# peterWon/D-LIOM

Measured on AMD Instinct MI355X. Metric: scans/sec (64-beam x 1024 pts -> 10 cm 3D submap), higher is better.
Workload: dtype f32 transforms + u16 voxels/u64 sums (rtcsm), f64 (ceres); 1 GPU; config2 W-dense: 64x1024 scan, all returns matched (adaptive voxel filters neutralised), RTCSM3D + CeresScanMatcher3D(hi+lo) + insertion(hi+lo); N_hi=65536, N_lo=65536, C=35937, linear_window=1, angular_window=5, rescored_candidates_last=2, box_kernel_variant=0, map_scans=20, grids_inserted_into=2, parallelism=replicas x1

## Files before the change

### d-liom_amd/csrc/rtcsm3d.hip

```cpp
#include <algorithm>
#include <cmath>
#include <cstdlib>
#include <cstring>
#include <type_traits>
#include <vector>

#include <dlfcn.h>
#include <rccl/rccl.h>

#include "device_common.h"
#include "host_math.h"
#include "probability_values.h"
#include "score_box.h"

namespace dliom {

constexpr int kBlock = 256;

template <int PPT, bool WIDE = false>
__global__ __launch_bounds__(kBlock) void rtcsm_score_kernel(
    GridView g, const float* __restrict__ px, const float* __restrict__ py,
    const float* __restrict__ pz, const float4* __restrict__ rot, int R, int r_first, int r_last,
    const float* __restrict__ trans, int T, int rots_per_block,
    unsigned long long* __restrict__ sums) {
  extern __shared__ unsigned block_sum[];
  float x[PPT], y[PPT], z[PPT];
#pragma unroll
  for (int k = 0; k < PPT; ++k) {
    const int i = (blockIdx.x * PPT + k) * kBlock + threadIdx.x;
    x[k] = px[i];
    y[k] = py[i];
    z[k] = pz[i];
  }
  const int r_begin = r_first + blockIdx.y * rots_per_block;
  const int r_end = min(r_begin + rots_per_block, r_last);
  const int lane = threadIdx.x & 63;
  const float inv = g.inv_resolution;
  typedef typename std::conditional<WIDE, unsigned long long, unsigned>::type idx_t;
  const idx_t sentinel = static_cast<idx_t>(1) << (3 * g.log2_leaves);
  const unsigned lb = static_cast<unsigned>(g.log2_leaves);
  for (int r = r_begin; r < r_end; ++r) {
    for (int j = threadIdx.x; j < T; j += kBlock) block_sum[j] = 0u;
    __syncthreads();
    const float4 qq = rot[r];
    const Quat4 q{qq.x, qq.y, qq.z, qq.w};
    float rx[PPT], ry[PPT], rz[PPT];
#pragma unroll
    for (int k = 0; k < PPT; ++k) rotate_point(q, x[k], y[k], z[k], rx[k], ry[k], rz[k]);
#pragma unroll 1
    for (int j = 0; j < T; ++j) {
      const float tx = trans[3 * j], ty = trans[3 * j + 1], tz = trans[3 * j + 2];
      idx_t tix[PPT];
      unsigned cel[PPT];
#pragma unroll
      for (int k = 0; k < PPT; ++k) {
        const float cx = rx[k] + tx, cy = ry[k] + ty, cz = rz[k] + tz;
        bool near = false;
        int ix = cell_fast(cx, inv, &near);
        int iy = cell_fast(cy, inv, &near);
        int iz = cell_fast(cz, inv, &near);
        if (__builtin_expect(near, 0)) {
          ix = cell_of(cx, g.resolution);
          iy = cell_of(cy, g.resolution);
          iz = cell_of(cz, g.resolution);
        }
        const unsigned sx = static_cast<unsigned>(ix + g.half);
        const unsigned sy = static_cast<unsigned>(iy + g.half);
        const unsigned sz = static_cast<unsigned>(iz + g.half);
        const bool inside = (sx | sy | sz) < g.grid_size;
        const idx_t t = (((static_cast<idx_t>(sz >> 3) << lb) | (sy >> 3)) << lb) | (sx >> 3);
        tix[k] = inside ? t : sentinel;
        cel[k] = ((sz & 7u) << 6) | ((sy & 7u) << 3) | (sx & 7u);
      }
#pragma unroll
      for (int k = 0; k < PPT; ++k) tix[k] = g.table[tix[k]];
#pragma unroll
      for (int k = 0; k < PPT; ++k) cel[k] = g.pool[(static_cast<size_t>(tix[k]) << 9) | cel[k]];
      unsigned a = 0;
#pragma unroll
      for (int k = 0; k < PPT; ++k) a += max(cel[k] & 0x7FFFu, 1u);
      const unsigned total = wave_sum_lane63(a);
      if (lane == 63) atomicAdd(&block_sum[j], total);
    }
    __syncthreads();
    for (int j = threadIdx.x; j < T; j += kBlock)
      atomicAdd(&sums[static_cast<size_t>(j) * R + r], static_cast<unsigned long long>(block_sum[j]));
  }
}

template <int TC, int P>
__global__ __launch_bounds__(kBlock) void rtcsm_score_rot_kernel(
    GridView g, const float* __restrict__ px, const float* __restrict__ py,
    const float* __restrict__ pz, int points_per_chunk, const float4* __restrict__ rot, int R,
    int r_first, int r_last, const float4* __restrict__ trans4, int T,
    unsigned long long* __restrict__ sums) {
  extern __shared__ float4 lds_trans[];
  __shared__ unsigned lds_acc[TC][kBlock];
  for (int j = threadIdx.x; j < T; j += kBlock) lds_trans[j] = trans4[j];
  __syncthreads();
  const int r = r_first + blockIdx.x * kBlock + threadIdx.x;
  const bool active = r < r_last;
  const float4 qq = rot[active ? r : r_first];
  const Quat4 q{qq.x, qq.y, qq.z, qq.w};
  const float inv = g.inv_resolution;
  const unsigned sentinel = 1u << (3 * g.log2_leaves);
  const unsigned lb = static_cast<unsigned>(g.log2_leaves);
  const int p_begin = blockIdx.y * points_per_chunk;
  const int p_end = p_begin + points_per_chunk;
  for (int jc = 0; jc < T; jc += TC) {
    const int tc = min(TC, T - jc);
    for (int jj = 0; jj < tc; ++jj) lds_acc[jj][threadIdx.x] = 0u;
#pragma unroll 1
    for (int i = p_begin; i < p_end; i += P) {
      float rx[P], ry[P], rz[P];
#pragma unroll
      for (int k = 0; k < P; ++k) rotate_point(q, px[i + k], py[i + k], pz[i + k], rx[k], ry[k], rz[k]);
#pragma unroll 1
      for (int jj = 0; jj < tc; ++jj) {
        const float4 t = lds_trans[jc + jj];
        unsigned tix[P], cel[P];
#pragma unroll
        for (int k = 0; k < P; ++k) {
          const float cx = rx[k] + t.x, cy = ry[k] + t.y, cz = rz[k] + t.z;
          bool near = false;
          int ix = cell_fast(cx, inv, &near);
          int iy = cell_fast(cy, inv, &near);
          int iz = cell_fast(cz, inv, &near);
          if (__builtin_expect(near, 0)) {
            ix = cell_of(cx, g.resolution);
            iy = cell_of(cy, g.resolution);
            iz = cell_of(cz, g.resolution);
          }
          const unsigned sx = static_cast<unsigned>(ix + g.half);
          const unsigned sy = static_cast<unsigned>(iy + g.half);
          const unsigned sz = static_cast<unsigned>(iz + g.half);
          const bool inside = (sx | sy | sz) < g.grid_size;
          const unsigned tt = (((sz >> 3) << lb | (sy >> 3)) << lb) | (sx >> 3);
          tix[k] = inside ? tt : sentinel;
          cel[k] = ((sz & 7u) << 6) | ((sy & 7u) << 3) | (sx & 7u);
        }
#pragma unroll
        for (int k = 0; k < P; ++k) tix[k] = g.table[tix[k]];
#pragma unroll
        for (int k = 0; k < P; ++k) cel[k] = g.pool[(tix[k] << 9) | cel[k]];
        unsigned a = 0;
#pragma unroll
        for (int k = 0; k < P; ++k) a += max(cel[k] & 0x7FFFu, 1u);
        atomicAdd(&lds_acc[jj][threadIdx.x], a);
      }
    }
    if (active) {
      for (int jj = 0; jj < tc; ++jj)
        atomicAdd(&sums[static_cast<size_t>(jc + jj) * R + r],
                  static_cast<unsigned long long>(lds_acc[jj][threadIdx.x]));
    }
  }
}

__device__ __forceinline__ int cvt_flr(float y) {
  int r;
  asm("v_cvt_flr_i32_f32 %0, %1" : "=v"(r) : "v"(y));
  return r;
}

constexpr int kDenseMaxBlock = 256;

struct DenseDomain {
  int lo;
  int size;
  int n_real;
  float pad[3];
};

template <bool CLAMP>
__global__ __launch_bounds__(kDenseMaxBlock) void rtcsm_score_dense_kernel(
    GridView g, DenseDomain dom, const float* __restrict__ px, const float* __restrict__ py,
    const float* __restrict__ pz, int points_per_chunk, int point_chunks,
    int rot_groups, const float4* __restrict__ rot, int R, int r_first, int r_last,
    const float4* __restrict__ trans4, int T, int t_chunk, unsigned long long* __restrict__ sums) {
  constexpr int P = 8;
  const int bs = blockDim.x;
  const int xcd = blockIdx.x & 7, slot = blockIdx.x >> 3;
  const int rot_group = slot % rot_groups;
  const int chunk_id = (slot / rot_groups) * 8 + xcd;
  if (chunk_id >= point_chunks) return;
  extern __shared__ float4 lds_dyn[];
  float4* lds_trans = lds_dyn;
  unsigned* lds_off = reinterpret_cast<unsigned*>(lds_dyn + T);
  const int S = g.dense_stride;
  const int TS = dom.size;
  unsigned* lds_acc = lds_off + 3 * TS;
  for (int j = threadIdx.x; j < T; j += bs) lds_trans[j] = trans4[j];
  {
    const unsigned B = static_cast<unsigned>(g.dense_bricks);
    for (int c = threadIdx.x; c < TS; c += bs) {
      const unsigned m = static_cast<unsigned>(min(max(c + dom.lo, 0), S - 1));
      const unsigned h = m >> 2, l = m & 3u;
      lds_off[c] = h * 128u + l * 2u;
      lds_off[TS + c] = h * B * 128u + l * 8u;
      lds_off[2 * TS + c] = h * B * B * 128u + l * 32u;
    }
  }
  __syncthreads();
  const int r = r_first + rot_group * bs + threadIdx.x;
  const bool active = r < r_last;
  const float4 qq = rot[active ? r : r_first];
  const Quat4 q{qq.x, qq.y, qq.z, qq.w};
  const float inv = g.inv_resolution;
  const float K = static_cast<float>(g.half + 1 - dom.lo) + 0.5f;
  const float band = 2.2f * static_cast<float>(TS) * 5.9604645e-8f;
  const float lim = static_cast<float>(TS - 1) + 0.5f;
  const int to_table = g.half + 1 - dom.lo;
  const int p_begin = chunk_id * points_per_chunk;
  const int p_end = p_begin + points_per_chunk;
  for (int jc = blockIdx.y * t_chunk; jc < T; jc += t_chunk * gridDim.y) {
    const int tc = min(t_chunk, T - jc);
    for (int jj = 0; jj < tc; ++jj) lds_acc[jj * bs + threadIdx.x] = 0u;
#pragma unroll 1
    for (int i = p_begin; i < p_end; i += P) {
      float rx[P], ry[P], rz[P];
#pragma unroll
      for (int k = 0; k < P; ++k) {
        const bool real = CLAMP || i + k < dom.n_real;
        rotate_point(q, real ? px[i + k] : dom.pad[0], real ? py[i + k] : dom.pad[1], real ? pz[i + k] : dom.pad[2],
                     rx[k], ry[k], rz[k]);
      }
#pragma unroll 1
      for (int jj = 0; jj < tc; ++jj) {
        const float4 t = lds_trans[jc + jj];
        unsigned ox[P], oy[P], oz[P];
        float lo[P], hi[P];
#pragma unroll
        for (int k = 0; k < P; ++k) {
          const float zx = __builtin_fmaf(rx[k] + t.x, inv, K), zy = __builtin_fmaf(ry[k] + t.y, inv, K),
                      zz = __builtin_fmaf(rz[k] + t.z, inv, K);
          const float fx = __builtin_amdgcn_fractf(zx), fy = __builtin_amdgcn_fractf(zy),
                      fz = __builtin_amdgcn_fractf(zz);
          lo[k] = fminf(fminf(fx, fy), fz);
          hi[k] = fmaxf(fmaxf(fx, fy), fz);
          if (CLAMP) {
            ox[k] = lds_off[cvt_flr(__builtin_amdgcn_fmed3f(zx, 0.f, lim))];
            oy[k] = lds_off[TS + cvt_flr(__builtin_amdgcn_fmed3f(zy, 0.f, lim))];
            oz[k] = lds_off[2 * TS + cvt_flr(__builtin_amdgcn_fmed3f(zz, 0.f, lim))];
          } else {
            ox[k] = lds_off[cvt_flr(zx)];
            oy[k] = lds_off[TS + cvt_flr(zy)];
            oz[k] = lds_off[2 * TS + cvt_flr(zz)];
          }
        }
        float m = lo[0], M = hi[0];
#pragma unroll
        for (int k = 1; k < P; ++k) {
          m = fminf(m, lo[k]);
          M = fmaxf(M, hi[k]);
        }
        if (__builtin_expect(m <= band || M >= 1.f - band, 0)) {
#pragma unroll
          for (int k = 0; k < P; ++k) {
            if (lo[k] <= band || hi[k] >= 1.f - band) {
              ox[k] = lds_off[min(max(cell_of(rx[k] + t.x, g.resolution) + to_table, 0), TS - 1)];
              oy[k] = lds_off[TS + min(max(cell_of(ry[k] + t.y, g.resolution) + to_table, 0), TS - 1)];
              oz[k] = lds_off[2 * TS + min(max(cell_of(rz[k] + t.z, g.resolution) + to_table, 0), TS - 1)];
            }
          }
        }
        unsigned v[P];
#pragma unroll
        for (int k = 0; k < P; ++k)
          v[k] = *reinterpret_cast<const unsigned short*>(reinterpret_cast<const char*>(g.dense) + (ox[k] + oy[k] + oz[k]));
        unsigned a = 0;
#pragma unroll
        for (int k = 0; k < P; ++k) a += v[k];
        atomicAdd(&lds_acc[jj * bs + threadIdx.x], a);
      }
    }
    if (active) {
      for (int jj = 0; jj < tc; ++jj)
        atomicAdd(&sums[static_cast<size_t>(jc + jj) * R + r],
                  static_cast<unsigned long long>(lds_acc[jj * bs + threadIdx.x]));
    }
  }
}

struct BoundParams {
  double a;
  double b;
  double delta;
  double wt, wr;
  int n;
  int n_pad;
  int R, T;
  int r_first, r_last;
};

__device__ double seq_sum_error_bound(int n, double U) {
  double err = 0.0;
  long long i = 0;
  for (int k = -4; k < 64 && i < n; ++k) {
    const double top = ldexp(1.0, k + 1);
    long long last;
    if (U < top) {
      last = n;
    } else {
      last = static_cast<long long>(floor(top / 0.93)) - 1;
      if (last > n) last = n;
    }
    if (last > i) {
      err += 0.5 * ldexp(1.0, k - 23) * static_cast<double>(last - i);
      i = last;
    }
  }
  return err;
}

__device__ __forceinline__ float next_up(float f) { return __uint_as_float(__float_as_uint(f) + 1u); }
__device__ __forceinline__ float next_down(float f) {
  const unsigned u = __float_as_uint(f);
  return u == 0u ? 0.f : __uint_as_float(u - 1u);
}

__global__ void rtcsm_bounds_kernel(const unsigned long long* __restrict__ sums, long long C,
                                    const float* __restrict__ t_norm, const float* __restrict__ r_angle,
                                    BoundParams p, float* __restrict__ lo, float* __restrict__ hi,
                                    unsigned* __restrict__ best_lo_bits) {
  const long long c = static_cast<long long>(blockIdx.x) * blockDim.x + threadIdx.x;
  const bool in_range = c < C;
  const int j = in_range ? static_cast<int>(c / p.R) : 0, r = in_range ? static_cast<int>(c % p.R) : 0;
  const bool mine = in_range && r >= p.r_first && r < p.r_last;
  float flo = 0.f, fhi = -1.f;
  if (mine) {
  const double s = static_cast<double>(sums[c] - static_cast<unsigned long long>(p.n_pad));
  const double mid = p.a * s + p.b * p.n;
  const double slack = p.delta * p.n + 1e-9 * mid;
  double sum_lo = mid - slack, sum_hi = mid + slack;
  const double U = sum_hi * (1.0 + 1.0 / 32.0);
  const double e = seq_sum_error_bound(p.n, U);
  if (sum_hi + e > U || p.n > (1 << 19)) {
    flo = 0.f;
    fhi = 3.0e38f;
  } else {
    sum_lo -= e;
    sum_hi += e;
    const double arg = static_cast<double>(t_norm[j]) * p.wt + static_cast<double>(r_angle[r]) * p.wr;
    const double pen = exp(-(arg * arg));
    const float nf = static_cast<float>(p.n);
    float qlo = next_down(next_down(static_cast<float>(sum_lo))) / nf;
    float qhi = next_up(next_up(static_cast<float>(sum_hi))) / nf;
    qlo = next_down(qlo);
    qhi = next_up(qhi);
    flo = next_down(next_down(static_cast<float>(static_cast<double>(qlo) * pen * (1.0 - 1e-9))));
    fhi = next_up(next_up(static_cast<float>(static_cast<double>(qhi) * pen * (1.0 + 1e-9))));
    if (!(flo > 0.f)) flo = 0.f;
  }
  }
  if (in_range) {
    lo[c] = flo;
    hi[c] = fhi;
  }
  unsigned best = __float_as_uint(flo);
#pragma unroll
  for (int off = 32; off > 0; off >>= 1) best = max(best, static_cast<unsigned>(__shfl_xor(static_cast<int>(best), off, 64)));
  if ((threadIdx.x & 63) == 0 && best != 0u) atomicMax(best_lo_bits, best);
}

__global__ void rtcsm_select_kernel(const float* __restrict__ hi, long long C,
                                    const unsigned* __restrict__ best_lo_bits,
                                    unsigned* __restrict__ count, unsigned* __restrict__ list) {
  const long long c = static_cast<long long>(blockIdx.x) * blockDim.x + threadIdx.x;
  if (c >= C) return;
  const float best_lo = __uint_as_float(*best_lo_bits);
  if (hi[c] >= best_lo) {
    const unsigned k = atomicAdd(count, 1u);
    list[k] = static_cast<unsigned>(c);
  }
}

__global__ void probe_cells_kernel(Quat4 q, float tx, float ty, float tz, const float* __restrict__ px,
                                   const float* __restrict__ py, const float* __restrict__ pz, int n,
                                   float resolution, int* __restrict__ out) {
  const int i = blockIdx.x * blockDim.x + threadIdx.x;
  if (i >= n) return;
  float rx, ry, rz;
  rotate_point(q, px[i], py[i], pz[i], rx, ry, rz);
  out[3 * i] = cell_of(rx + tx, resolution);
  out[3 * i + 1] = cell_of(ry + ty, resolution);
  out[3 * i + 2] = cell_of(rz + tz, resolution);
}

struct Candidates {
  dliom_rtcsm_window w;
  PoseF init;
  std::vector<QF> rot;
  std::vector<QF> rot_raw;
  std::vector<float> r_angle;
  std::vector<F3> trans;
  std::vector<float> t_norm;
};

static void compute_window(const dliom_rtcsm_options& o, float resolution, float cloud_max_norm_value,
                           dliom_rtcsm_window* w) {
  w->linear_window_size = static_cast<int>(std::lround(o.linear_search_window / resolution));
  float max_scan_range = 3.f * resolution;
  max_scan_range = std::max(cloud_max_norm_value, max_scan_range);
  const float kSafetyMargin = 1.f - 1e-3f;
  const float res2 = resolution * (resolution * 1.f);
  const float range2 = max_scan_range * (max_scan_range * 1.f);
  w->angular_step_size = kSafetyMargin * std::acos(1.f - res2 / (2.f * range2));
  w->angular_window_size =
      static_cast<int>(std::lround(o.angular_search_window / w->angular_step_size));
  w->max_scan_range = max_scan_range;
  const int64_t tl = 2 * static_cast<int64_t>(w->linear_window_size) + 1;
  const int64_t ta = 2 * static_cast<int64_t>(w->angular_window_size) + 1;
  w->num_translations = tl * tl * tl;
  w->num_rotations = ta * ta * ta;
  w->num_candidates = w->num_translations * w->num_rotations;
}

static void generate_candidates(const dliom_rtcsm_options& o, float resolution, float max_norm,
                                const double init7[7], Candidates* c) {
  compute_window(o, resolution, max_norm, &c->w);
  c->init.t = F3{static_cast<float>(init7[0]), static_cast<float>(init7[1]), static_cast<float>(init7[2])};
  c->init.q = QF{static_cast<float>(init7[3]), static_cast<float>(init7[4]),
                 static_cast<float>(init7[5]), static_cast<float>(init7[6])};
  const int L = c->w.linear_window_size, A = c->w.angular_window_size;
  const float step = c->w.angular_step_size;
  struct RotCache {
    int A = -1;
    float step = 0.f;
    std::vector<QF> rot_raw;
    std::vector<float> r_angle;
  };
  static thread_local RotCache cache;
  if (cache.A != A || cache.step != step) {
    cache.A = A;
    cache.step = step;
    cache.rot_raw.clear();
    cache.r_angle.clear();
    cache.rot_raw.reserve(c->w.num_rotations);
    cache.r_angle.reserve(c->w.num_rotations);
    for (int rz = -A; rz <= A; ++rz)
      for (int ry = -A; ry <= A; ++ry)
        for (int rx = -A; rx <= A; ++rx) {
          const QF q = angle_axis_to_quaternion(F3{rx * step, ry * step, rz * step});
          cache.rot_raw.push_back(q);
          cache.r_angle.push_back(rotation_angle(q));
        }
  }
  c->rot_raw = cache.rot_raw;
  c->r_angle = cache.r_angle;
  c->rot.resize(cache.rot_raw.size());
  for (size_t i = 0; i < cache.rot_raw.size(); ++i) c->rot[i] = qnormalized(qmul(c->init.q, cache.rot_raw[i]));
  c->trans.clear();
  c->t_norm.clear();
  for (int z = -L; z <= L; ++z)
    for (int y = -L; y <= L; ++y)
      for (int x = -L; x <= L; ++x) {
        const F3 t{x * resolution, y * resolution, z * resolution};
        c->t_norm.push_back(norm3(t));
        c->trans.push_back(add3(qrot(c->init.q, t), c->init.t));
      }
}

struct DeviceCandidates {
  float4* rot;
  float* trans;
  float4* trans4;
  float* t_norm;
  float* r_angle;
  const float4* rot_src;
};

static bool prep_add(PrepArgs* prep, void* dst, const void* src, size_t bytes, unsigned value) {
  if (prep == nullptr || prep->n >= kMaxPrepJobs || (bytes & 3u) != 0 || (reinterpret_cast<uintptr_t>(dst) & 15u) != 0 ||
      (reinterpret_cast<uintptr_t>(src) & 15u) != 0 || bytes / 16 > 0xFFFFFFFFull)
    return false;
  PrepJob& j = prep->job[prep->n++];
  j.dst = static_cast<uint4*>(dst);
  j.src = static_cast<const uint4*>(src);
  j.vec = static_cast<unsigned>(bytes / 16);
  j.tail_words = static_cast<unsigned>((bytes % 16) / 4);
  j.value = value;
  return true;
}
__global__ __launch_bounds__(256) void rtcsm_prep_kernel(PrepArgs a) { prep_block(a, blockIdx.x, gridDim.x, threadIdx.x, blockDim.x); }
static int prep_flush(dliom_ctx* ctx, PrepArgs* prep) {
  if (prep == nullptr || prep->n == 0) return DLIOM_OK;
  unsigned most = 1;
  for (int j = 0; j < prep->n; ++j) most = std::max(most, prep->job[j].vec);
  hipLaunchKernelGGL(rtcsm_prep_kernel, dim3(std::min(512u, (most + 255u) / 256u)), dim3(256), 0, ctx->stream, *prep);
  DLIOM_HIP_TRY(hipGetLastError());
  prep->n = 0;
  return DLIOM_OK;
}

static int upload_candidates(dliom_ctx* ctx, const Candidates& c, DeviceCandidates* d, PrepArgs* prep = nullptr) {
  const size_t R = c.rot.size(), T = c.trans.size();
  const size_t Tpad = T;
  const size_t bytes_rot = align256(R * 16);
  const size_t bytes_trans = align256(Tpad * 12);
  const size_t bytes_tn = align256(T * 4);
  const size_t bytes_ra = align256(R * 4);
  const size_t bytes_t4 = align256(T * 16);
  const size_t total = bytes_rot + bytes_trans + bytes_tn + bytes_ra + bytes_t4;
  DLIOM_TRY(ctx->cand.reserve(total));
  std::vector<char> host(total, 0);
  float* hr = reinterpret_cast<float*>(host.data());
  for (size_t i = 0; i < R; ++i) {
    hr[4 * i] = c.rot[i].w;
    hr[4 * i + 1] = c.rot[i].x;
    hr[4 * i + 2] = c.rot[i].y;
    hr[4 * i + 3] = c.rot[i].z;
  }
  float* ht = reinterpret_cast<float*>(host.data() + bytes_rot);
  for (size_t i = 0; i < Tpad; ++i) {
    const F3& t = c.trans[std::min(i, T - 1)];
    ht[3 * i] = t.x;
    ht[3 * i + 1] = t.y;
    ht[3 * i + 2] = t.z;
  }
  std::memcpy(host.data() + bytes_rot + bytes_trans, c.t_norm.data(), T * 4);
  std::memcpy(host.data() + bytes_rot + bytes_trans + bytes_tn, c.r_angle.data(), R * 4);
  float* h4 = reinterpret_cast<float*>(host.data() + bytes_rot + bytes_trans + bytes_tn + bytes_ra);
  for (size_t i = 0; i < T; ++i) {
    h4[4 * i] = c.trans[i].x;
    h4[4 * i + 1] = c.trans[i].y;
    h4[4 * i + 2] = c.trans[i].z;
    h4[4 * i + 3] = 0.f;
  }
  char* base = static_cast<char*>(ctx->cand.p);
  d->rot_src = reinterpret_cast<const float4*>(base);
  if (total <= kPinRtcsmCandidates.bytes) {
    void* staged = pinned_at(ctx, kPinRtcsmCandidates);
    std::memcpy(staged, host.data(), total);
    if (prep_add(prep, base, staged, total, 0u))
      d->rot_src = static_cast<const float4*>(staged);
    else
      DLIOM_HIP_TRY(hipMemcpyAsync(base, staged, total, hipMemcpyHostToDevice, ctx->stream));
  } else {
    DLIOM_HIP_TRY(hipMemcpyAsync(base, host.data(), total, hipMemcpyHostToDevice, ctx->stream));
    DLIOM_HIP_TRY(hipStreamSynchronize(ctx->stream));
  }
  d->rot = reinterpret_cast<float4*>(base);
  d->trans = reinterpret_cast<float*>(base + bytes_rot);
  d->t_norm = reinterpret_cast<float*>(base + bytes_rot + bytes_trans);
  d->r_angle = reinterpret_cast<float*>(base + bytes_rot + bytes_trans + bytes_tn);
  d->trans4 = reinterpret_cast<float4*>(base + bytes_rot + bytes_trans + bytes_tn + bytes_ra);
  return DLIOM_OK;
}

static int env_int(const char* name, int fallback) { return tuning_int(name, fallback); }

static int launch_score_box(dliom_ctx* ctx, const dliom_cloud& cloud, const GridView& g, const Candidates& c,
                            const DeviceCandidates& d, int r_first, int r_last, unsigned long long* d_sums,
                            unsigned* d_error, PrepArgs* prep) {
  using namespace box;
  const int R = static_cast<int>(c.w.num_rotations), T = static_cast<int>(c.w.num_translations);
  const int n = static_cast<int>(cloud.n);
  static const int forced_variant = env_int("DLIOM_BOX_VARIANT", -1);
  const auto padded = [T](int tc) { return ((T + tc - 1) / tc) * tc; };
  const int variant = forced_variant >= 0 && forced_variant <= 2
                          ? forced_variant
                          : (T <= kTC ? 0 : (0.87 * padded(kTCWide) < 0.9 * padded(kTC) ? 2 : 1));
  const int TC = variant == 2 ? kTCWide : kTC;
  static const int forced_cells = env_int("DLIOM_BOX_CELLS", 0);
  const int cells = forced_cells > 0 ? forced_cells : (variant == 0 ? 14336 : 21000);
  static const int forced_chunk = env_int("DLIOM_BOX_CHUNK", 0);
  const int chunk_pts = forced_chunk > 0 ? forced_chunk : (variant == 0 ? kCostChunk : kCostChunkBig);
  const double res = static_cast<double>(g.resolution);
  const int passes = (T + TC - 1) / TC;
  double tmax = 0.0;
  for (const F3& t : c.trans) tmax = std::max(tmax, static_cast<double>(std::max(std::fabs(t.x), std::max(std::fabs(t.y), std::fabs(t.z)))));
  const double rmax = static_cast<double>(cloud.max_norm) / res + 1.0;
  const double qmax = rmax + tmax / res + 1.0;
  if (!std::isfinite(qmax) || qmax > 16500.0) return (ctx->last_box_refusal = DLIOM_BOX_REFUSED_RANGE, DLIOM_ERR_CAPACITY);
  std::vector<Pass> pass(static_cast<size_t>(passes));
  std::vector<float> tau(static_cast<size_t>(passes) * TC * 4, 0.f);
  double taumax = 0.0;
  for (int tp = 0; tp < passes; ++tp) {
    const int j0 = tp * TC, tc = std::min(TC, T - j0);
    for (int a = 0; a < 3; ++a) {
      double lo = 1e300, hi = -1e300;
      for (int j = j0; j < j0 + tc; ++j) {
        const double v = a == 0 ? c.trans[j].x : (a == 1 ? c.trans[j].y : c.trans[j].z);
        lo = std::min(lo, v);
        hi = std::max(hi, v);
      }
      taumax = std::max(taumax, (hi - lo) * 0.5 / res + 1.0);
    }
  }
  if (rmax + taumax + 130.0 > 1000.0) return (ctx->last_box_refusal = DLIOM_BOX_REFUSED_RANGE, DLIOM_ERR_CAPACITY);
  const double e16 = 1.0 + (2.0 * qmax + rmax + taumax) / 256.0;
  const int B = static_cast<int>(std::ceil(e16 + 0.25));
  const int s_units = B;
  const double u = 1.0 / 65536.0;
  for (int tp = 0; tp < passes; ++tp) {
    Pass& ps = pass[static_cast<size_t>(tp)];
    ps.j0 = tp * TC;
    ps.tc = std::min(TC, T - ps.j0);
    ps.pad[0] = ps.pad[1] = 0;
    for (int a = 0; a < 3; ++a) {
      auto comp = [&](int j) { return static_cast<double>(a == 0 ? c.trans[j].x : (a == 1 ? c.trans[j].y : c.trans[j].z)); };
      double lo = 1e300, hi = -1e300;
      for (int j = ps.j0; j < ps.j0 + ps.tc; ++j) {
        lo = std::min(lo, comp(j));
        hi = std::max(hi, comp(j));
      }
      const double tcen = 0.5 * (lo + hi);
      const double G = tcen / res + 128.5 + s_units * u;
      const double gi = std::floor(G);
      const double f = std::nearbyint((G - gi) * 16384.0) / 16384.0;
      ps.gi[a] = static_cast<int>(gi);
      ps.f[a] = static_cast<float>(f);
      ps.uc[a] = static_cast<float>(tcen / res + 0.5);
      double reach = 0.0;
      for (int jj = 0; jj < TC; ++jj) {
        const int j = ps.j0 + std::min(jj, ps.tc - 1);
        const double tv = comp(j) / res + 128.5 + s_units * u - (gi + f);
        const float tf = static_cast<float>(tv);
        tau[(static_cast<size_t>(tp) * TC + jj) * 4 + a] = tf;
        reach = std::max(reach, std::fabs(static_cast<double>(tf)));
      }
      ps.reach[a] = static_cast<float>(reach + 0.02 + qmax * std::ldexp(1.0, -22));
    }
  }
  std::vector<unsigned> bitmap(static_cast<size_t>(passes) * kBitmapWords, 0u);
  const unsigned thr_units = static_cast<unsigned>(s_units + B);
  for (int tp = 0; tp < passes; ++tp) {
    const Pass& ps = pass[static_cast<size_t>(tp)];
    for (int a = 0; a < 3; ++a) {
      unsigned* words = bitmap.data() + static_cast<size_t>(tp) * kBitmapWords + static_cast<size_t>(a) * (kBuckets / 32);
      for (int jj = 0; jj < ps.tc; ++jj) {
        const double tv = static_cast<double>(tau[(static_cast<size_t>(tp) * TC + jj) * 4 + a]);
        const double af = tv - std::floor(tv);
        const double L = -af - 1.5 * u, H = -af + (thr_units + 1.5) * u;
        const long long b0 = static_cast<long long>(std::floor(L * kBuckets)), b1 = static_cast<long long>(std::floor(H * kBuckets));
        for (long long b = b0; b <= b1; ++b) {
          const unsigned m = static_cast<unsigned>(((b % kBuckets) + kBuckets) % kBuckets);
          words[m >> 5] |= 1u << (m & 31u);
        }
      }
    }
  }
  {
    const double step = c.w.angular_step_size;
    const double a_lanes = (2.0 * c.w.angular_window_size + 1.0) * step;
    const double spread = a_lanes * 0.6 * cloud.max_norm / res;
    const double dim = spread + 2.0 * taumax + 8.0;
    if (dim > kMaxDim || dim * dim * (dim * 0.25) > cells) return (ctx->last_box_refusal = DLIOM_BOX_REFUSED_WINDOW, DLIOM_ERR_CAPACITY);
  }
  const int rot_groups_all = (r_last - r_first + 63) / 64;
  static const int forced_nw = env_int("DLIOM_BOX_NW", 0);
  const int nw = forced_nw >= 1 && forced_nw <= kWaves
                     ? std::min(forced_nw, rot_groups_all)
                     : std::min(rot_groups_all, kWaves);
  const int rot_blocks = (rot_groups_all + nw - 1) / nw;
  if (TC * sizeof(float4) + kBitmapWords * 4 + 16 + static_cast<size_t>(nw) * kListWords * 4 + static_cast<size_t>(cells) * 2 >
      160 * 1024)
    return (ctx->last_box_refusal = DLIOM_BOX_REFUSED_LDS, DLIOM_ERR_CAPACITY);
  struct GroupCache {
    int A = -1, r_first = -1, r_last = -1, nw = 0;
    float step = 0.f;
    std::vector<Group> groups;
  };
  static thread_local GroupCache gcache;
  const bool gcache_hit = gcache.A == c.w.angular_window_size && gcache.step == c.w.angular_step_size &&
                          gcache.r_first == r_first && gcache.r_last == r_last && gcache.nw == nw;
  std::vector<Group>& groups = gcache.groups;
  if (!gcache_hit) {
    gcache.A = -1;
    groups.assign(static_cast<size_t>(rot_blocks), Group());
  }
  for (size_t gi = 0; !gcache_hit && gi < groups.size(); ++gi) {
    Group& gr = groups[gi];
    const int r0 = r_first + static_cast<int>(gi) * nw * 64;
    const int cnt = std::max(0, std::min(nw * 64, r_last - r0));
    gr.c_lane = cnt / 2;
    gr.theta2 = 0.f;
    for (int a = 0; a < 3; ++a) gr.dc[a] = gr.hd[a] = 0.f;
    if (cnt <= 0) {
      gr.c_lane = 0;
      continue;
    }
    auto qd = [&](int r, double q[4]) {
      const QF& f = c.rot_raw[static_cast<size_t>(r)];
      const double nn = std::sqrt(double(f.w) * f.w + double(f.x) * f.x + double(f.y) * f.y + double(f.z) * f.z);
      q[0] = f.w / nn; q[1] = f.x / nn; q[2] = f.y / nn; q[3] = f.z / nn;
    };
    double qc[4];
    qd(r0 + gr.c_lane, qc);
    double lo3[3] = {1e300, 1e300, 1e300}, hi3[3] = {-1e300, -1e300, -1e300}, th = 0.0;
    for (int l = 0; l < cnt; ++l) {
      double q[4];
      qd(r0 + l, q);
      const double a0 = qc[0], a1 = -qc[1], a2 = -qc[2], a3 = -qc[3];
      double dq[4] = {a0 * q[0] - a1 * q[1] - a2 * q[2] - a3 * q[3], a0 * q[1] + a1 * q[0] + a2 * q[3] - a3 * q[2],
                      a0 * q[2] - a1 * q[3] + a2 * q[0] + a3 * q[1], a0 * q[3] + a1 * q[2] - a2 * q[1] + a3 * q[0]};
      if (dq[0] < 0) for (double& v : dq) v = -v;
      const double vn = std::sqrt(dq[1] * dq[1] + dq[2] * dq[2] + dq[3] * dq[3]);
      const double ang = 2.0 * std::atan2(vn, dq[0]);
      const double k = vn > 1e-300 ? ang / vn : 2.0;
      const double dv[3] = {k * dq[1], k * dq[2], k * dq[3]};
      th = std::max(th, ang);
      for (int a = 0; a < 3; ++a) {
        lo3[a] = std::min(lo3[a], dv[a]);
        hi3[a] = std::max(hi3[a], dv[a]);
      }
    }
    if (th > 0.3) return (ctx->last_box_refusal = DLIOM_BOX_REFUSED_WINDOW, DLIOM_ERR_CAPACITY);
    for (int a = 0; a < 3; ++a) {
      gr.dc[a] = static_cast<float>(0.5 * (lo3[a] + hi3[a]));
      gr.hd[a] = static_cast<float>(0.5 * (hi3[a] - lo3[a]) * 1.0001 + 1e-7);
    }
    gr.theta2 = static_cast<float>(0.51 * th * th * 1.01 + 1e-9);
  }
  gcache.A = c.w.angular_window_size;
  gcache.step = c.w.angular_step_size;
  gcache.r_first = r_first;
  gcache.r_last = r_last;
  gcache.nw = nw;
  struct SpanGuard {
    dliom_ctx* c;
    int span;
    ~SpanGuard() { c->end_span(span); }
  } span_guard{ctx, ctx->begin_span(DLIOM_KERNEL_RTCSM_SCORE)};
  const size_t tau_bytes = align256(tau.size() * 4);
  const size_t pass_only_bytes = align256(pass.size() * sizeof(Pass));
  const size_t group_bytes = align256(groups.size() * sizeof(Group));
  const size_t bitmap_bytes = align256(bitmap.size() * 4);
  const size_t pass_bytes = pass_only_bytes + group_bytes + bitmap_bytes;
  DLIOM_TRY(ctx->box_tables.reserve(tau_bytes + pass_bytes));
  char* base = static_cast<char*>(ctx->box_tables.p);
  const Group* group_src = reinterpret_cast<const Group*>(base + tau_bytes + pass_only_bytes);
  if (tau_bytes + pass_bytes <= kPinBoxTables.bytes) {
    char* h = pinned_at<char>(ctx, kPinBoxTables);
    std::memcpy(h, tau.data(), tau.size() * 4);
    std::memcpy(h + tau_bytes, pass.data(), pass.size() * sizeof(Pass));
    std::memcpy(h + tau_bytes + pass_only_bytes, groups.data(), groups.size() * sizeof(Group));
    std::memcpy(h + tau_bytes + pass_only_bytes + group_bytes, bitmap.data(), bitmap.size() * 4);
    if (prep_add(prep, base, h, tau_bytes + pass_bytes, 0u))
      group_src = reinterpret_cast<const Group*>(h + tau_bytes + pass_only_bytes);
    else
      DLIOM_HIP_TRY(hipMemcpyAsync(base, h, tau_bytes + pass_bytes, hipMemcpyHostToDevice, ctx->stream));
  } else {
    DLIOM_HIP_TRY(hipMemcpyAsync(base, tau.data(), tau.size() * 4, hipMemcpyHostToDevice, ctx->stream));
    DLIOM_HIP_TRY(hipMemcpyAsync(base + tau_bytes, pass.data(), pass.size() * sizeof(Pass), hipMemcpyHostToDevice, ctx->stream));
    DLIOM_HIP_TRY(hipMemcpyAsync(base + tau_bytes + pass_only_bytes, groups.data(), groups.size() * sizeof(Group),
                                 hipMemcpyHostToDevice, ctx->stream));
    DLIOM_HIP_TRY(hipMemcpyAsync(base + tau_bytes + pass_only_bytes + group_bytes, bitmap.data(), bitmap.size() * 4,
                                 hipMemcpyHostToDevice, ctx->stream));
    DLIOM_HIP_TRY(hipStreamSynchronize(ctx->stream));
  }
  Params p;
  p.tau = reinterpret_cast<const float4*>(base);
  p.pass = reinterpret_cast<const Pass*>(base + tau_bytes);
  p.group = reinterpret_cast<const Group*>(base + tau_bytes + pass_only_bytes);
  p.bitmap = reinterpret_cast<const unsigned*>(base + tau_bytes + pass_only_bytes + group_bytes);
  p.trans = d.trans;
  p.rot = d.rot;
  p.sums = d_sums;
  p.error = d_error;
  p.R = R;
  p.r_first = r_first;
  p.r_last = r_last;
  p.T = T;
  p.passes = passes;
  p.n = n;
  p.chunk = std::min(kMaxChunk, std::max(4, chunk_pts & ~3));
  p.order = p.chunk == kCostChunk ? cloud.d_chunk_order : (p.chunk == kCostChunkBig ? cloud.d_chunk_order_big : nullptr);
  p.point_chunks = (n + p.chunk - 1) / p.chunk;
  const int rot_groups = (r_last - r_first + 63) / 64;
  p.rot_groups = rot_groups;
  p.rot_blocks = rot_blocks;
  p.nw = nw;
  p.thr = thr_units;
  p.cells = cells;
  static const int split_points = env_int("DLIOM_BOX_SPLIT", 1);
  p.split_points = split_points;
#ifdef DLIOM_EXPERIMENTS
  static const int box_debug = env_int("DLIOM_BOX_DEBUG", 0);
  p.debug = box_debug;
  if (box_debug & 512) p.order = nullptr;
#else
  p.debug = 0;
#endif
  const size_t lds = TC * sizeof(float4) + kBitmapWords * 4 + 16 + static_cast<size_t>(nw) * kListWords * 4 +
                     static_cast<size_t>(cells) * 2;
  if (lds > 160 * 1024) return (ctx->last_box_refusal = DLIOM_BOX_REFUSED_LDS, DLIOM_ERR_CAPACITY);
  typedef void (*BoxKernel)(GridView, Params, const float*, const float*, const float*);
  const BoxKernel kernel = variant == 0 ? rtcsm_score_box_kernel : (variant == 1 ? rtcsm_score_box_kernel_w3 : rtcsm_score_box_kernel_wide);
  const unsigned attr_bit = variant == 0 ? kFuncAttrScoreBox : (variant == 1 ? kFuncAttrScoreBoxW3 : kFuncAttrScoreBoxWide);
  if ((ctx->func_attr_set & attr_bit) == 0u) {
    DLIOM_HIP_TRY(hipFuncSetAttribute(reinterpret_cast<const void*>(kernel), hipFuncAttributeMaxDynamicSharedMemorySize, 160 * 1024));
    ctx->func_attr_set |= attr_bit;
  }
  ctx->last_box_variant = variant;
  static thread_local size_t resident_lds = 0;
  static thread_local int resident = 0, resident_nw = 0, resident_variant = -1;
  if (resident_lds != lds || resident_nw != nw || resident_variant != variant) {
    resident_nw = nw;
    resident_variant = variant;
    DLIOM_HIP_TRY(hipOccupancyMaxActiveBlocksPerMultiprocessor(&resident, reinterpret_cast<const void*>(kernel), 64 * nw, lds));
    resident_lds = lds;
  }
  const int want_blocks = std::max(1, resident) * ctx->num_cus;
  int slot_quads = std::max(1, want_blocks / std::max(1, rot_blocks * passes));
  slot_quads = std::min(slot_quads, p.point_chunks);
  p.slots = slot_quads;
  p.units = passes * rot_blocks;
  DLIOM_TRY(ctx->box_counters.reserve(static_cast<size_t>(passes) * rot_blocks * 4 + 256));
  if (!prep_add(prep, ctx->box_counters.p, nullptr, static_cast<size_t>(passes) * rot_blocks * 4, 0u))
    DLIOM_HIP_TRY(hipMemsetAsync(ctx->box_counters.p, 0, static_cast<size_t>(passes) * rot_blocks * 4, ctx->stream));
  p.counters = ctx->box_counters.as<unsigned>();
  p.ext_stride = static_cast<int>(cloud.n_padded);
  DLIOM_TRY(ctx->box_extents.reserve(static_cast<size_t>(rot_blocks) * 6 * static_cast<size_t>(cloud.n_padded) * 4));
  p.ext = ctx->box_extents.as<float>();
  {
    PrepArgs none;
    none.n = 0;
    const PrepArgs& jobs = prep != nullptr ? *prep : none;
    const unsigned prep_rows = jobs.n > 0 ? 1u : 0u;
    hipLaunchKernelGGL(rtcsm_box_extent_kernel, dim3(static_cast<unsigned>((n + 255) / 256), static_cast<unsigned>(rot_blocks) + prep_rows),
                       dim3(256), 0, ctx->stream, p, g.inv_resolution, cloud.d_xs, cloud.d_ys, cloud.d_zs, ctx->box_extents.as<float>(),
                       group_src, d.rot_src, jobs);
    if (prep != nullptr) prep->n = 0;
  }
  const unsigned blocks = static_cast<unsigned>(slot_quads) * passes * rot_blocks;
  hipLaunchKernelGGL(kernel, dim3(blocks), dim3(64 * nw), lds, ctx->stream, g, p, cloud.d_xs, cloud.d_ys, cloud.d_zs);
  DLIOM_HIP_TRY(hipGetLastError());
#ifdef DLIOM_TEST_HOOKS
  if (ctx->tuning[DLIOM_TUNE_RESERVED_TEST_HOOK] == 1) {
    ctx->tuning[DLIOM_TUNE_RESERVED_TEST_HOOK] = 0;
    DLIOM_HIP_TRY(hipMemsetAsync(static_cast<char*>(ctx->box_error.p) + 4, 1, 1, ctx->stream));
  }
#endif
  return DLIOM_OK;
}

constexpr int kScoreTargetBlocks = 8192;

static int launch_score_dense(dliom_ctx* ctx, const dliom_cloud& cloud, const GridView& g, const Candidates& c,
                              const DeviceCandidates& d, int r_first, int r_last, unsigned long long* d_sums,
                              int64_t* processed) {
  const int R = static_cast<int>(c.w.num_rotations), T = static_cast<int>(c.w.num_translations);
  const int n = static_cast<int>(cloud.n);
  const int Rs = r_last - r_first;
  const size_t trans_lds = static_cast<size_t>(T) * 16;
  if (trans_lds > 100 * 1024) return DLIOM_ERR_INVALID_ARGUMENT;
  int bs = kDenseMaxBlock;
  for (int cand = kDenseMaxBlock; cand >= 64; cand -= 64)
    if ((Rs + cand - 1) / cand * cand < (Rs + bs - 1) / bs * bs) bs = cand;
  if (static_cast<int64_t>((Rs + bs - 1) / bs) * ((n + 63) / 64) < 256) bs = 64;
  const int rot_groups = (Rs + bs - 1) / bs;
  int chunk = 4096;
  while (chunk > 8 && static_cast<int64_t>(rot_groups) * ((n + chunk - 1) / chunk) < kScoreTargetBlocks) chunk >>= 1;
  const int point_chunks = (n + chunk - 1) / chunk;
  *processed = static_cast<int64_t>(point_chunks) * chunk;
  DenseDomain dom;
  dom.lo = 0;
  dom.size = g.dense_stride;
  dom.n_real = n;
  dom.pad[0] = dom.pad[1] = dom.pad[2] = kPadCoordinate;
  bool clamp = true;
  {
    float tmax = 0.f, t_init = norm3(c.init.t);
    for (const F3& t : c.trans) tmax = std::max(tmax, std::max(std::fabs(t.x), std::max(std::fabs(t.y), std::fabs(t.z))));
    const float res = g.resolution;
    const double reach = (static_cast<double>(cloud.max_norm) + tmax) / res + 3.0;
    const double theta_max = 1.7321 * (c.w.angular_window_size + 1) * c.w.angular_step_size * 1.01 + 1e-4;
    const double rho = (g.half + 64) * static_cast<double>(res) + t_init;
    const double m_cells = 8.0 + std::ceil((theta_max * rho + (c.w.linear_window_size + 1) * res * 1.7321) / res);
    const double hi_cell = std::max(reach, g.half + 2.0 * m_cells);
    const int lo_i = std::min(0, g.half + 1 - static_cast<int>(std::ceil(hi_cell)));
    const int hi_i = std::max(g.dense_stride, g.half + 1 + static_cast<int>(std::ceil(hi_cell)) + 1);
    if (m_cells <= 64.0 && hi_i - lo_i <= 1024 && std::isfinite(reach)) {
      clamp = false;
      dom.lo = lo_i;
      dom.size = hi_i - lo_i;
      const F3 w{static_cast<float>((g.half + m_cells) * res) - c.init.t.x, -c.init.t.y, -c.init.t.z};
      const QF qi{c.init.q.w, -c.init.q.x, -c.init.q.y, -c.init.q.z};
      const F3 p = qrot(qi, w);
      dom.pad[0] = p.x;
      dom.pad[1] = p.y;
      dom.pad[2] = p.z;
    }
  }
  const size_t fixed_lds = trans_lds + static_cast<size_t>(dom.size) * 12;
  const size_t acc_budget = fixed_lds < 34 * 1024 ? 36 * 1024 - fixed_lds : 2 * 1024;
  int t_chunk = std::max(4, std::min(std::min(T, 27), static_cast<int>(acc_budget / (static_cast<size_t>(bs) * 4))));
  const int chunks_per_xcd = (point_chunks + 7) / 8;
  int t_slices = 1;
  const int base_blocks = 8 * chunks_per_xcd * rot_groups;
  if (base_blocks < 512 && T > 1) {
    const int want = std::min(T, (1024 + base_blocks - 1) / base_blocks);
    t_chunk = std::min(t_chunk, (T + want - 1) / want);
    t_slices = (T + t_chunk - 1) / t_chunk;
  }
  const size_t lds = fixed_lds + static_cast<size_t>(t_chunk) * bs * 4;
  const auto kernel = clamp ? &rtcsm_score_dense_kernel<true> : &rtcsm_score_dense_kernel<false>;
  const int span = ctx->begin_span(DLIOM_KERNEL_RTCSM_SCORE);
  hipLaunchKernelGGL(kernel, dim3(base_blocks, t_slices), dim3(bs), lds, ctx->stream, g, dom, cloud.d_xs, cloud.d_ys,
                     cloud.d_zs, chunk, point_chunks, rot_groups, d.rot, R, r_first, r_last, d.trans4, T, t_chunk, d_sums);
  ctx->end_span(span);
  return DLIOM_OK;
}

static int launch_score_rot(dliom_ctx* ctx, const dliom_cloud& cloud, const GridView& g, const Candidates& c,
                            const DeviceCandidates& d, int r_first, int r_last, unsigned long long* d_sums,
                            int64_t* processed) {
  const int R = static_cast<int>(c.w.num_rotations), T = static_cast<int>(c.w.num_translations);
  const int n = static_cast<int>(cloud.n);
  const size_t lds = static_cast<size_t>(T) * 16;
  if (lds > 100 * 1024) return DLIOM_ERR_INVALID_ARGUMENT;
  const int rot_groups = (r_last - r_first + kBlock - 1) / kBlock;
  int chunk = 4096;
  while (chunk > 64 && static_cast<int64_t>(rot_groups) * ((n + chunk - 1) / chunk) < kScoreTargetBlocks) chunk >>= 1;
  const int point_chunks = (n + chunk - 1) / chunk;
  *processed = static_cast<int64_t>(point_chunks) * chunk;
  const auto kernel = T == 1 ? &rtcsm_score_rot_kernel<1, 4> : &rtcsm_score_rot_kernel<27, 8>;
  const int span = ctx->begin_span(DLIOM_KERNEL_RTCSM_SCORE);
  hipLaunchKernelGGL(kernel, dim3(rot_groups, point_chunks), dim3(kBlock), lds, ctx->stream, g, cloud.d_xs, cloud.d_ys,
                     cloud.d_zs, chunk, d.rot, R, r_first, r_last, d.trans4, T, d_sums);
  ctx->end_span(span);
  return DLIOM_OK;
}

static int launch_score_point(dliom_ctx* ctx, const dliom_cloud& cloud, const GridView& g, const Candidates& c,
                              const DeviceCandidates& d, int r_first, int r_last, unsigned long long* d_sums,
                              int64_t* processed) {
  const int R = static_cast<int>(c.w.num_rotations), T = static_cast<int>(c.w.num_translations);
  const int n = static_cast<int>(cloud.n);
  const int Rs = r_last - r_first;
  int ppt = n >= 32 * 1024 ? 8 : (n >= 8 * 1024 ? 4 : (n >= 2048 ? 2 : 1));
  while (ppt > 1 && (cloud.n_padded % (static_cast<int64_t>(kBlock) * ppt)) != 0) ppt >>= 1;
  const int point_tiles = (n + kBlock * ppt - 1) / (kBlock * ppt);
  int rot_tiles = std::max(1, std::min(Rs, (kScoreTargetBlocks + point_tiles - 1) / point_tiles));
  const int rots_per_block = (Rs + rot_tiles - 1) / rot_tiles;
  rot_tiles = (Rs + rots_per_block - 1) / rots_per_block;
  const size_t lds = static_cast<size_t>(T) * sizeof(unsigned);
  if (lds > 150 * 1024) return DLIOM_ERR_INVALID_ARGUMENT;
  const bool wide = g.log2_leaves > 10;
  const int lane_pts = wide ? (ppt >= 4 ? 4 : 1) : ppt;
  const int tile = kBlock * lane_pts;
  const int tiles = (n + tile - 1) / tile;
  *processed = static_cast<int64_t>(tiles) * tile;
  auto kernel = &rtcsm_score_kernel<1>;
  if (wide) kernel = lane_pts == 4 ? &rtcsm_score_kernel<4, true> : &rtcsm_score_kernel<1, true>;
  else if (lane_pts == 8) kernel = &rtcsm_score_kernel<8>;
  else if (lane_pts == 4) kernel = &rtcsm_score_kernel<4>;
  else if (lane_pts == 2) kernel = &rtcsm_score_kernel<2>;
  const int span = ctx->begin_span(DLIOM_KERNEL_RTCSM_SCORE);
  hipLaunchKernelGGL(kernel, dim3(tiles, rot_tiles), dim3(kBlock), lds, ctx->stream, g, cloud.d_xs, cloud.d_ys, cloud.d_zs,
                     d.rot, R, r_first, r_last, d.trans, T, rots_per_block, d_sums);
  ctx->end_span(span);
  return DLIOM_OK;
}

static int run_score_volume(dliom_ctx* ctx, const dliom_cloud& cloud, const dliom_grid* grid,
                            const Candidates& c, int r_first, int r_last, DeviceCandidates* d,
                            unsigned long long** d_sums, int64_t* pad_processed, const FillJob* also_fill = nullptr) {
  PrepArgs prep;
  prep.n = 0;
  DLIOM_TRY(upload_candidates(ctx, c, d, &prep));
  const int64_t C = c.w.num_candidates;
  DLIOM_TRY(ctx->sums.reserve(static_cast<size_t>(C) * 8));
  *d_sums = ctx->sums.as<unsigned long long>();
  {
    FillJob fills[2] = {{*d_sums, static_cast<size_t>(C) * 8, 0u}, {nullptr, 0, 0u}};
    int nf = 1;
    if (also_fill != nullptr) fills[nf++] = *also_fill;
    for (int k = 0; k < nf; ++k)
      if (!prep_add(&prep, fills[k].p, nullptr, fills[k].bytes, fills[k].value)) DLIOM_TRY(fill_multi(ctx, &fills[k], 1));
  }
  const int T = static_cast<int>(c.w.num_translations);
  const int n = static_cast<int>(cloud.n);
  int mapping = ctx->tuning[DLIOM_TUNE_SCORE_KERNEL];
  ctx->last_box_refusal = mapping == 3 ? DLIOM_BOX_RAN : DLIOM_BOX_NOT_REQUESTED;
  if (ctx->force_dense_score && mapping > 2) {
    mapping = 2;
    ctx->last_box_refusal = DLIOM_BOX_REFUSED_FLAGGED;
  }
  ctx->last_score_used_box = false;
  if (mapping >= 2) {
    const float res = grid->resolution;
    const int centre[3] = {static_cast<int>(std::lround(c.init.t.x / res)), static_cast<int>(std::lround(c.init.t.y / res)),
                           static_cast<int>(std::lround(c.init.t.z / res))};
    const double reach_cells = static_cast<double>(cloud.max_norm) / res + (c.w.linear_window_size + 1) * 1.7321 + 4.0;
    const int radius = reach_cells < 1.0e6 ? static_cast<int>(std::ceil(reach_cells)) : (1 << 20);
    if (const_cast<dliom_grid*>(grid)->ensure_dense_for(centre, radius) != DLIOM_OK) {
      if (mapping == 3) ctx->last_box_refusal = DLIOM_BOX_REFUSED_NO_MIRROR;
      mapping = 1;
    }
  }
  const bool windowed = grid->dense_windowed;
  if (windowed && mapping == 2) mapping = 1;
  const GridView g = grid->view();
  DLIOM_TRY(ensure_morton(ctx, &cloud));
  if (g.log2_leaves > 10 && mapping >= 1) {
    if (mapping == 3) ctx->last_box_refusal = DLIOM_BOX_REFUSED_NO_MIRROR;
    mapping = 0;
  }
  if (mapping == 3) {
    const double pairs = static_cast<double>(C) * static_cast<double>(n);
    int s3 = DLIOM_ERR_CAPACITY;
    ctx->last_box_refusal = DLIOM_BOX_REFUSED_SMALL;
    if (T >= 8 && pairs >= std::ldexp(1.0, 24)) {
      ctx->last_box_refusal = DLIOM_BOX_RAN;
#ifdef DLIOM_EXPERIMENTS
      constexpr size_t kBoxErrorBytes = 256 + 4096 * 32;
#else
      constexpr size_t kBoxErrorBytes = 256;
#endif
      DLIOM_TRY(ctx->box_error.reserve(kBoxErrorBytes));
      if (!ctx->box_error_zeroed) {
        DLIOM_HIP_TRY(hipMemsetAsync(ctx->box_error.p, 0, kBoxErrorBytes, ctx->stream));
        ctx->box_error_zeroed = true;
      }
      s3 = launch_score_box(ctx, cloud, g, c, *d, r_first, r_last, *d_sums, ctx->box_error.as<unsigned>(), &prep);
    }
    if (s3 == DLIOM_OK) {
      *pad_processed = 0;
      ctx->last_score_used_box = true;
      ctx->last_score_mapping = 3;
      return DLIOM_OK;
    }
    if (s3 != DLIOM_ERR_CAPACITY) return s3;
    mapping = windowed ? 1 : 2;
  }
  DLIOM_TRY(prep_flush(ctx, &prep));
  ctx->last_score_mapping = mapping;
  int64_t processed = 0;
  if (mapping == 2)
    DLIOM_TRY(launch_score_dense(ctx, cloud, g, c, *d, r_first, r_last, *d_sums, &processed));
  else if (mapping == 1)
    DLIOM_TRY(launch_score_rot(ctx, cloud, g, c, *d, r_first, r_last, *d_sums, &processed));
  else
    DLIOM_TRY(launch_score_point(ctx, cloud, g, c, *d, r_first, r_last, *d_sums, &processed));
  DLIOM_HIP_TRY(hipGetLastError());
  *pad_processed = processed - n;
  return DLIOM_OK;
}

struct LutModel {
  double a, b, delta;
};
static const LutModel& lut_model() {
  static const LutModel m = [] {
    LutModel r;
    r.a = static_cast<double>(kValueToProbabilityScale);
    r.b = static_cast<double>(kValueToProbabilityOffset);
    double d = std::fabs(static_cast<double>(kUnknownProbability) - (r.a * 1.0 + r.b));
    for (int v = 1; v < 32768; ++v) {
      const float f = v * kValueToProbabilityScale + kValueToProbabilityOffset;
      d = std::max(d, std::fabs(static_cast<double>(f) - (r.a * v + r.b)));
    }
    r.delta = d * 1.0000001 + 1e-12;
    return r;
  }();
  return m;
}

struct RtcsmState {
  dliom_rtcsm_options o;
  Candidates c;
  DeviceCandidates d;
  dliom_cloud cloud;
  const dliom_grid* grid = nullptr;
  int r_first = 0, r_last = 0;
  unsigned long long* d_sums = nullptr;
  float* d_hi = nullptr;
  unsigned* d_list = nullptr;
  unsigned* d_ctrs = nullptr;
  float best_score = -1.f;
  int64_t best_c = -1;
  bool active = false;
  double init7[7] = {0, 0, 0, 1, 0, 0, 0};
  int shard = 0, num_shards = 1;
  bool used_box = false;
};

static int box_overflowed(dliom_ctx* ctx, unsigned err1, bool* overflow) {
  *overflow = err1 != 0u;
  if (*overflow)
    DLIOM_HIP_TRY(hipMemsetAsync(static_cast<char*>(ctx->box_error.p) + 4, 0, 4, ctx->stream));
  return DLIOM_OK;
}

static RtcsmState* state_of(dliom_ctx* ctx) {
  if (ctx->rtcsm_state == nullptr) {
    ctx->rtcsm_state = new RtcsmState;
    ctx->rtcsm_state_free = [](void* p) { delete static_cast<RtcsmState*>(p); };
  }
  return static_cast<RtcsmState*>(ctx->rtcsm_state);
}

static int match_begin(dliom_ctx* ctx, const dliom_rtcsm_options* o, const double init7[7],
                       const dliom_cloud& cloud, const dliom_grid* grid, int shard, int num_shards,
                       unsigned* local_best_lo_bits) {
  if (cloud.n <= 0) return DLIOM_ERR_EMPTY_CLOUD;
  if (cloud.n > (1 << 27) || num_shards < 1 || shard < 0 || shard >= num_shards)
    return DLIOM_ERR_INVALID_ARGUMENT;
  RtcsmState* st = state_of(ctx);
  st->active = false;
  st->o = *o;
  st->cloud = cloud;
  st->grid = grid;
  std::memcpy(st->init7, init7, sizeof st->init7);
  st->shard = shard;
  st->num_shards = num_shards;
  st->used_box = false;
  Candidates& c = st->c;
  generate_candidates(*o, grid->resolution, cloud.max_norm, init7, &c);
  const int64_t C = c.w.num_candidates;
  const int R = static_cast<int>(c.w.num_rotations), T = static_cast<int>(c.w.num_translations);
  if (C <= 0 || C > (int64_t{1} << 31)) return DLIOM_ERR_INVALID_ARGUMENT;
  st->r_first = static_cast<int>(static_cast<int64_t>(R) * shard / num_shards);
  st->r_last = static_cast<int>(static_cast<int64_t>(R) * (shard + 1) / num_shards);

  const size_t bytes_f = align256(static_cast<size_t>(C) * 4);
  DLIOM_TRY(ctx->bounds.reserve(3 * bytes_f + 256));
  char* bb = static_cast<char*>(ctx->bounds.p);
  float* d_lo = reinterpret_cast<float*>(bb);
  st->d_hi = reinterpret_cast<float*>(bb + bytes_f);
  st->d_list = reinterpret_cast<unsigned*>(bb + 2 * bytes_f);
  st->d_ctrs = reinterpret_cast<unsigned*>(bb + 3 * bytes_f);
  const FillJob zero_ctrs{st->d_ctrs, 8, 0u};
  if (st->r_last <= st->r_first) DLIOM_TRY(fill_multi(ctx, &zero_ctrs, 1));
  if (st->r_last > st->r_first) {
    int64_t pad_processed = 0;
    DLIOM_TRY(run_score_volume(ctx, cloud, grid, c, st->r_first, st->r_last, &st->d, &st->d_sums,
                               &pad_processed, &zero_ctrs));
    st->used_box = ctx->last_score_used_box;
    const LutModel& lm = lut_model();
    BoundParams bp;
    bp.a = lm.a;
    bp.b = lm.b;
    bp.delta = lm.delta;
    bp.wt = o->translation_delta_cost_weight;
    bp.wr = o->rotation_delta_cost_weight;
    bp.n = static_cast<int>(cloud.n);
    bp.n_pad = static_cast<int>(pad_processed);
    bp.R = R;
    bp.T = T;
    bp.r_first = st->r_first;
    bp.r_last = st->r_last;
    const unsigned cblocks = static_cast<unsigned>((C + 255) / 256);
    const int span = ctx->begin_span(DLIOM_KERNEL_RTCSM_SELECT);
    hipLaunchKernelGGL(rtcsm_bounds_kernel, dim3(cblocks), dim3(256), 0, ctx->stream, st->d_sums,
                       static_cast<long long>(C), st->d.t_norm, st->d.r_angle, bp, d_lo, st->d_hi,
                       st->d_ctrs);
    ctx->end_span(span);
    DLIOM_HIP_TRY(hipGetLastError());
  }
  if (local_best_lo_bits != nullptr) {
    unsigned* h_err = pinned_at<unsigned>(ctx, kPinBoxErrorWord);
    *h_err = 0u;
    DLIOM_HIP_TRY(hipMemcpyAsync(local_best_lo_bits, st->d_ctrs, 4, hipMemcpyDeviceToHost, ctx->stream));
    if (st->used_box)
      DLIOM_HIP_TRY(hipMemcpyAsync(h_err, static_cast<char*>(ctx->box_error.p) + 4, 4, hipMemcpyDeviceToHost, ctx->stream));
    DLIOM_HIP_TRY(hipStreamSynchronize(ctx->stream));
    bool overflow = false;
    DLIOM_TRY(box_overflowed(ctx, *h_err, &overflow));
    if (overflow && !ctx->force_dense_score) {
      ctx->force_dense_score = true;
      const dliom_rtcsm_options o_copy = st->o;
      const int s = match_begin(ctx, &o_copy, init7, cloud, grid, shard, num_shards, local_best_lo_bits);
      ctx->force_dense_score = false;
      return s;
    }
  }
  st->active = true;
  return DLIOM_OK;
}

static int match_finish(dliom_ctx* ctx, const unsigned* global_best_lo_bits, uint64_t* local_best_packed) {
  RtcsmState* st = state_of(ctx);
  if (!st->active) return DLIOM_ERR_INVALID_ARGUMENT;
  const dliom_rtcsm_options* o = &st->o;
  const Candidates& c = st->c;
  const int64_t C = c.w.num_candidates;
  const int R = static_cast<int>(c.w.num_rotations);
  const dliom_cloud& cloud = st->cloud;
  st->best_score = -1.f;
  st->best_c = -1;
  unsigned K = 0;
  if (st->r_last > st->r_first) {
    if (global_best_lo_bits != nullptr) {
      DLIOM_HIP_TRY(hipMemcpyAsync(st->d_ctrs, global_best_lo_bits, 4, hipMemcpyHostToDevice, ctx->stream));
    }
    const unsigned cblocks = static_cast<unsigned>((C + 255) / 256);
    int span = ctx->begin_span(DLIOM_KERNEL_RTCSM_SELECT);
    hipLaunchKernelGGL(rtcsm_select_kernel, dim3(cblocks), dim3(256), 0, ctx->stream, st->d_hi,
                       static_cast<long long>(C), st->d_ctrs, st->d_ctrs + 1, st->d_list);
    ctx->end_span(span);
    DLIOM_HIP_TRY(hipGetLastError());
  }
  constexpr unsigned kSpecK = 8;
  std::vector<unsigned> list;
  std::vector<float> ksums;
  if (st->r_last > st->r_first) {
    static_assert((2 + 2 * kSpecK + 1) * 4 <= kPinMatchReadback.bytes, "the read-back fits its region");
    unsigned* h_ctrs = pinned_at<unsigned>(ctx, kPinMatchReadback);
    unsigned* h_list = h_ctrs + 2;
    float* h_sums = reinterpret_cast<float*>(h_ctrs + 2 + kSpecK);
    auto rescore = [&](unsigned count, const unsigned* d_count, size_t list_offset) -> int {
      DLIOM_TRY(ctx->rescore.reserve(align256(static_cast<size_t>(count) * 4)));
      const int span = ctx->begin_span(DLIOM_KERNEL_RTCSM_RESCORE);
      const int s = launch_sequential_sums(ctx, sequential_sum_method(cloud.n), st->grid->view(), cloud, st->d.rot, R, st->d.trans,
                                           st->d_list + list_offset, d_count, count, &ctx->misc, ctx->rescore.as<float>());
      ctx->end_span(span);
      return s;
    };
    DLIOM_TRY(rescore(kSpecK, st->d_ctrs + 1, 0));
    unsigned* h_err = h_ctrs + 2 + 2 * kSpecK;
    *h_err = 0u;
    const bool want_err = st->used_box && global_best_lo_bits == nullptr;
    const GatherJob back[4] = {{st->d_ctrs, 2}, {st->d_list, kSpecK}, {ctx->rescore.p, kSpecK},
                               {static_cast<char*>(ctx->box_error.p) + 4, 1}};
    DLIOM_TRY(gather_and_wait(ctx, back, want_err ? 4 : 3, h_ctrs));
    {
      bool overflow = false;
      DLIOM_TRY(box_overflowed(ctx, *h_err, &overflow));
      if (overflow && !ctx->force_dense_score) {
        ctx->force_dense_score = true;
        const dliom_rtcsm_options o_copy = st->o;
        const dliom_cloud cloud_copy = st->cloud;
        double init_copy[7];
        std::memcpy(init_copy, st->init7, sizeof init_copy);
        int s = match_begin(ctx, &o_copy, init_copy, cloud_copy, st->grid, st->shard, st->num_shards, nullptr);
        if (s == DLIOM_OK) s = match_finish(ctx, nullptr, local_best_packed);
        ctx->force_dense_score = false;
        return s;
      }
    }
    K = h_ctrs[1];
    const unsigned first = std::min(K, kSpecK);
    list.assign(h_list, h_list + first);
    ksums.assign(h_sums, h_sums + first);
    if (K > kSpecK) {
      const unsigned rest = K - kSpecK;
      DLIOM_TRY(rescore(rest, nullptr, kSpecK));
      list.resize(K);
      ksums.resize(K);
      DLIOM_HIP_TRY(hipMemcpyAsync(list.data() + kSpecK, st->d_list + kSpecK, static_cast<size_t>(rest) * 4,
                                   hipMemcpyDeviceToHost, ctx->stream));
      DLIOM_HIP_TRY(hipMemcpyAsync(ksums.data() + kSpecK, ctx->rescore.p, static_cast<size_t>(rest) * 4,
                                   hipMemcpyDeviceToHost, ctx->stream));
      DLIOM_HIP_TRY(hipStreamSynchronize(ctx->stream));
    }
  }
  if (K > 0) {
    const int n = static_cast<int>(cloud.n);
    for (unsigned k = 0; k < K; ++k) {
      const int64_t cc = list[k];
      const int j = static_cast<int>(cc / R), r = static_cast<int>(cc % R);
      float score = ksums[k];
      score /= static_cast<float>(n);
      const double arg = c.t_norm[j] * o->translation_delta_cost_weight +
                         c.r_angle[r] * o->rotation_delta_cost_weight;
      score *= std::exp(-(arg * (arg * 1.0)));
      if (score > st->best_score || (score == st->best_score && cc < st->best_c)) {
        st->best_score = score;
        st->best_c = cc;
      }
    }
  }
  ctx->last_rtcsm.window = c.w;
  ctx->last_rtcsm.num_points = cloud.n;
  ctx->last_rtcsm.num_rescored = K;
  ctx->last_rtcsm.score_kernel = ctx->last_score_mapping;
  ctx->last_rtcsm.box_kernel_status = ctx->last_box_refusal;
  ctx->last_rtcsm.box_kernel_variant = ctx->last_box_refusal == DLIOM_BOX_RAN ? ctx->last_box_variant : -1;
  ctx->last_rtcsm.best_index = st->best_c;
  if (local_best_packed != nullptr) {
    uint64_t packed = 0;
    if (st->best_c >= 0 && st->best_score > 0.f) {
      uint32_t bits;
      std::memcpy(&bits, &st->best_score, 4);
      packed = (static_cast<uint64_t>(bits) << 32) | (0xFFFFFFFFull - static_cast<uint64_t>(st->best_c));
    }
    *local_best_packed = packed;
  }
  return DLIOM_OK;
}

static int match_decode(dliom_ctx* ctx, uint64_t best_packed, double out7[7], float* out_score) {
  RtcsmState* st = state_of(ctx);
  if (!st->active) return DLIOM_ERR_INVALID_ARGUMENT;
  if (best_packed == 0) return DLIOM_ERR_SCORE_NOT_POSITIVE;
  const Candidates& c = st->c;
  const int R = static_cast<int>(c.w.num_rotations);
  const uint32_t bits = static_cast<uint32_t>(best_packed >> 32);
  const int64_t best_c = static_cast<int64_t>(0xFFFFFFFFull - (best_packed & 0xFFFFFFFFull));
  if (best_c < 0 || best_c >= c.w.num_candidates) return DLIOM_ERR_INVALID_ARGUMENT;
  float score;
  std::memcpy(&score, &bits, 4);
  const int j = static_cast<int>(best_c / R), r = static_cast<int>(best_c % R);
  out7[0] = c.trans[j].x;
  out7[1] = c.trans[j].y;
  out7[2] = c.trans[j].z;
  out7[3] = c.rot[r].w;
  out7[4] = c.rot[r].x;
  out7[5] = c.rot[r].y;
  out7[6] = c.rot[r].z;
  *out_score = score;
  ctx->last_rtcsm.best_index = best_c;
  return DLIOM_OK;
}

static int match_impl(dliom_ctx* ctx, const dliom_rtcsm_options* o, const double init7[7],
                      const dliom_cloud& cloud, const dliom_grid* grid, double out7[7],
                      float* out_score) {
  DLIOM_TRY(match_begin(ctx, o, init7, cloud, grid, 0, 1, nullptr));
  uint64_t packed = 0;
  DLIOM_TRY(match_finish(ctx, nullptr, &packed));
  return match_decode(ctx, packed, out7, out_score);
}

}

using namespace dliom;

extern "C" {

int dliom_rtcsm3d_window(const dliom_rtcsm_options* o, float resolution, const float* points_xyz,
                         int64_t n, dliom_rtcsm_window* w) {
  if (o == nullptr || w == nullptr || n < 0 || (n > 0 && points_xyz == nullptr))
    return DLIOM_ERR_INVALID_ARGUMENT;
  compute_window(*o, resolution, cloud_max_norm(points_xyz, n), w);
  return DLIOM_OK;
}

int dliom_rtcsm3d_match_cloud(dliom_ctx* ctx, const dliom_rtcsm_options* o, const double init7[7],
                              const dliom_cloud* cloud, const dliom_grid* grid, double out7[7],
                              float* score) {
  if (ctx == nullptr || o == nullptr || init7 == nullptr || cloud == nullptr || grid == nullptr ||
      out7 == nullptr || score == nullptr)
    return DLIOM_ERR_INVALID_ARGUMENT;
  DLIOM_HIP_TRY(hipSetDevice(ctx->device));
  return match_impl(ctx, o, init7, *cloud, grid, out7, score);
}

int dliom_rtcsm3d_match(dliom_ctx* ctx, const dliom_rtcsm_options* o, const double init7[7],
                        const float* points_xyz, int64_t n, const dliom_grid* grid, double out7[7],
                        float* score) {
  if (ctx == nullptr || o == nullptr || init7 == nullptr || grid == nullptr || out7 == nullptr ||
      score == nullptr || n < 0 || (n > 0 && points_xyz == nullptr))
    return DLIOM_ERR_INVALID_ARGUMENT;
  if (n == 0) return DLIOM_ERR_EMPTY_CLOUD;
  DLIOM_HIP_TRY(hipSetDevice(ctx->device));
  DLIOM_TRY(ctx->points.reserve(staged_cloud_bytes(n)));
  dliom_cloud cloud;
  DLIOM_TRY(stage_cloud(ctx, points_xyz, n, &cloud));
  return match_impl(ctx, o, init7, cloud, grid, out7, score);
}

int dliom_rtcsm3d_shard_begin(dliom_ctx* ctx, const dliom_rtcsm_options* o, const double init7[7],
                              const dliom_cloud* cloud, const dliom_grid* grid, int shard, int num_shards,
                              uint32_t* local_best_lower_bound_bits) {
  if (ctx == nullptr || o == nullptr || init7 == nullptr || cloud == nullptr || grid == nullptr ||
      local_best_lower_bound_bits == nullptr)
    return DLIOM_ERR_INVALID_ARGUMENT;
  DLIOM_HIP_TRY(hipSetDevice(ctx->device));
  return match_begin(ctx, o, init7, *cloud, grid, shard, num_shards, local_best_lower_bound_bits);
}

int dliom_rtcsm3d_shard_finish(dliom_ctx* ctx, uint32_t global_best_lower_bound_bits,
                               uint64_t* local_best_packed) {
  if (ctx == nullptr || local_best_packed == nullptr) return DLIOM_ERR_INVALID_ARGUMENT;
  DLIOM_HIP_TRY(hipSetDevice(ctx->device));
  return match_finish(ctx, &global_best_lower_bound_bits, local_best_packed);
}

int dliom_rtcsm3d_shard_decode(dliom_ctx* ctx, uint64_t global_best_packed, double pose_estimate[7],
                               float* score) {
  if (ctx == nullptr || pose_estimate == nullptr || score == nullptr) return DLIOM_ERR_INVALID_ARGUMENT;
  return match_decode(ctx, global_best_packed, pose_estimate, score);
}

static constexpr uint64_t kShardFailed = 0x7FFFFFFFFFFFFFFFull;
int dliom_rtcsm3d_match_sharded(dliom_ctx* ctx, const dliom_rtcsm_options* o, const double init7[7], const dliom_cloud* cloud,
                                const dliom_grid* grid, int shard, int num_shards, dliom_allreduce_max_u64 exchange,
                                void* user, double out7[7], float* score) {
  if (num_shards > 1 && exchange == nullptr) return DLIOM_ERR_INVALID_ARGUMENT;
  int local = ctx == nullptr || o == nullptr || init7 == nullptr || cloud == nullptr || grid == nullptr || out7 == nullptr ||
                      score == nullptr
                  ? DLIOM_ERR_INVALID_ARGUMENT
                  : DLIOM_OK;
  if (local == DLIOM_OK && hipSetDevice(ctx->device) != hipSuccess) local = DLIOM_ERR_HIP;
  uint64_t packed = 0;
  if (local == DLIOM_OK) local = match_begin(ctx, o, init7, *cloud, grid, shard, num_shards, nullptr);
  if (local == DLIOM_OK) local = match_finish(ctx, nullptr, &packed);
  if (local != DLIOM_OK) packed = kShardFailed;
  if (num_shards > 1 && exchange(&packed, user) != 0) return local != DLIOM_OK ? local : DLIOM_ERR_HIP;
  if (local != DLIOM_OK) return local;
  if (packed == kShardFailed) return DLIOM_ERR_PEER_FAILED;
  return match_decode(ctx, packed, out7, score);
}

}

namespace {
struct RcclApi {
  ncclResult_t (*CommCount)(const ncclComm_t, int*) = nullptr;
  ncclResult_t (*CommUserRank)(const ncclComm_t, int*) = nullptr;
  ncclResult_t (*AllReduce)(const void*, void*, size_t, ncclDataType_t, ncclRedOp_t, ncclComm_t, hipStream_t) = nullptr;
  bool ok = false;
};
const RcclApi& rccl_api() {
  static const RcclApi api = [] {
    RcclApi a;
    void* h = dlopen("librccl.so.1", RTLD_NOW | RTLD_GLOBAL);
    if (h == nullptr) h = dlopen("librccl.so", RTLD_NOW | RTLD_GLOBAL);
    if (h == nullptr) return a;
    a.CommCount = reinterpret_cast<decltype(a.CommCount)>(dlsym(h, "ncclCommCount"));
    a.CommUserRank = reinterpret_cast<decltype(a.CommUserRank)>(dlsym(h, "ncclCommUserRank"));
    a.AllReduce = reinterpret_cast<decltype(a.AllReduce)>(dlsym(h, "ncclAllReduce"));
    a.ok = a.CommCount != nullptr && a.CommUserRank != nullptr && a.AllReduce != nullptr;
    return a;
  }();
  return api;
}
struct RcclExchange {
  dliom_ctx* ctx;
  ncclComm_t comm;
};
int rccl_exchange(uint64_t* value, void* user) {
  RcclExchange* x = static_cast<RcclExchange*>(user);
  dliom_ctx* ctx = x->ctx;
  if (ctx->misc.reserve(256) != DLIOM_OK) return 1;
  uint64_t* d = ctx->misc.as<uint64_t>();
  uint64_t* h = pinned_at<uint64_t>(ctx, kPinRcclWord);
  *h = *value;
  const int span = ctx->begin_span(DLIOM_KERNEL_ALLREDUCE);
  bool ok = hipMemcpyAsync(d, h, 8, hipMemcpyHostToDevice, ctx->stream) == hipSuccess &&
            rccl_api().AllReduce(d, d, 1, ncclUint64, ncclMax, x->comm, ctx->stream) == ncclSuccess &&
            hipMemcpyAsync(h, d, 8, hipMemcpyDeviceToHost, ctx->stream) == hipSuccess;
  ctx->end_span(span);
  if (!ok) return 1;
  if (hipStreamSynchronize(ctx->stream) != hipSuccess) return 1;
  *value = *h;
  return 0;
}
}

extern "C" {

int dliom_rtcsm3d_match_sharded_rccl(dliom_ctx* ctx, const dliom_rtcsm_options* o, const double init7[7],
                                     const dliom_cloud* cloud, const dliom_grid* grid, void* nccl_comm, double out7[7],
                                     float* score) {
  if (ctx == nullptr || nccl_comm == nullptr) return DLIOM_ERR_INVALID_ARGUMENT;
  const RcclApi& api = rccl_api();
  if (!api.ok) {
    set_last_error("dlopen(librccl.so.1): RCCL not available", hipErrorSharedObjectInitFailed, __FILE__, __LINE__);
    return DLIOM_ERR_HIP;
  }
  int rank = 0, size = 1;
  ncclComm_t comm = static_cast<ncclComm_t>(nccl_comm);
  if (api.CommCount(comm, &size) != ncclSuccess || api.CommUserRank(comm, &rank) != ncclSuccess) return DLIOM_ERR_INVALID_ARGUMENT;
  RcclExchange x{ctx, comm};
  if (size == 1) {
    if (ctx == nullptr || o == nullptr || init7 == nullptr || cloud == nullptr || grid == nullptr || out7 == nullptr ||
        score == nullptr)
      return DLIOM_ERR_INVALID_ARGUMENT;
    int local = hipSetDevice(ctx->device) == hipSuccess ? DLIOM_OK : DLIOM_ERR_HIP;
    uint64_t packed = 0;
    if (local == DLIOM_OK) local = match_begin(ctx, o, init7, *cloud, grid, 0, 1, nullptr);
    if (local == DLIOM_OK) local = match_finish(ctx, nullptr, &packed);
    if (local != DLIOM_OK) packed = kShardFailed;
    if (rccl_exchange(&packed, &x) != 0) return local != DLIOM_OK ? local : DLIOM_ERR_HIP;
    if (local != DLIOM_OK) return local;
    return match_decode(ctx, packed, out7, score);
  }
  return dliom_rtcsm3d_match_sharded(ctx, o, init7, cloud, grid, rank, size, rccl_exchange, &x, out7, score);
}

int dliom_rtcsm3d_box_error(dliom_ctx* ctx, uint32_t* flags) {
  if (ctx == nullptr || flags == nullptr) return DLIOM_ERR_INVALID_ARGUMENT;
  *flags = 0;
  if (ctx->box_error.p == nullptr) return DLIOM_OK;
  DLIOM_HIP_TRY(hipSetDevice(ctx->device));
  DLIOM_HIP_TRY(hipMemcpyAsync(flags, ctx->box_error.p, 4, hipMemcpyDeviceToHost, ctx->stream));
  DLIOM_HIP_TRY(hipStreamSynchronize(ctx->stream));
  return DLIOM_OK;
}

#ifdef DLIOM_EXPERIMENTS
extern "C" int dliom_exp_box_stats(dliom_ctx* ctx, uint32_t out[8]) {
  if (ctx == nullptr || out == nullptr || ctx->box_error.p == nullptr) return DLIOM_ERR_INVALID_ARGUMENT;
  DLIOM_HIP_TRY(hipMemcpyAsync(out, static_cast<char*>(ctx->box_error.p) + 32, 32, hipMemcpyDeviceToHost, ctx->stream));
  DLIOM_HIP_TRY(hipMemsetAsync(static_cast<char*>(ctx->box_error.p) + 32, 0, 32, ctx->stream));
  DLIOM_HIP_TRY(hipStreamSynchronize(ctx->stream));
  return DLIOM_OK;
}
#endif

#ifdef DLIOM_EXPERIMENTS
extern "C" int dliom_exp_box_stamps(dliom_ctx* ctx, uint64_t* out, int workgroups) {
  if (ctx == nullptr || out == nullptr || ctx->box_error.p == nullptr || workgroups > 4096) return DLIOM_ERR_INVALID_ARGUMENT;
  DLIOM_HIP_TRY(hipMemcpyAsync(out, static_cast<char*>(ctx->box_error.p) + 256, static_cast<size_t>(workgroups) * 32,
                               hipMemcpyDeviceToHost, ctx->stream));
  DLIOM_HIP_TRY(hipStreamSynchronize(ctx->stream));
  return DLIOM_OK;
}
#endif

int dliom_rtcsm3d_last_stats(const dliom_ctx* ctx, dliom_rtcsm_stats* stats) {
  if (ctx == nullptr || stats == nullptr) return DLIOM_ERR_INVALID_ARGUMENT;
  *stats = ctx->last_rtcsm;
  return DLIOM_OK;
}

int dliom_rtcsm3d_score_volume(dliom_ctx* ctx, const dliom_rtcsm_options* o, const double init7[7],
                               const float* points_xyz, int64_t n, const dliom_grid* grid,
                               uint64_t* sums, int64_t capacity, int64_t* num_candidates) {
  if (ctx == nullptr || o == nullptr || init7 == nullptr || grid == nullptr ||
      num_candidates == nullptr || n <= 0 || points_xyz == nullptr)
    return DLIOM_ERR_INVALID_ARGUMENT;
  DLIOM_HIP_TRY(hipSetDevice(ctx->device));
  DLIOM_TRY(ctx->points.reserve(staged_cloud_bytes(n)));
  dliom_cloud cloud;
  DLIOM_TRY(stage_cloud(ctx, points_xyz, n, &cloud));
  Candidates c;
  generate_candidates(*o, grid->resolution, cloud.max_norm, init7, &c);
  *num_candidates = c.w.num_candidates;
  if (sums == nullptr) return DLIOM_OK;
  if (capacity < c.w.num_candidates) return DLIOM_ERR_CAPACITY;
  DeviceCandidates d;
  unsigned long long* d_sums = nullptr;
  int64_t pad_processed = 0;
  DLIOM_TRY(run_score_volume(ctx, cloud, grid, c, 0, static_cast<int>(c.w.num_rotations), &d, &d_sums,
                             &pad_processed));
  unsigned err1 = 0u;
  if (ctx->last_score_used_box)
    DLIOM_HIP_TRY(hipMemcpyAsync(&err1, static_cast<char*>(ctx->box_error.p) + 4, 4, hipMemcpyDeviceToHost, ctx->stream));
  DLIOM_HIP_TRY(hipMemcpyAsync(sums, d_sums, static_cast<size_t>(c.w.num_candidates) * 8,
                               hipMemcpyDeviceToHost, ctx->stream));
  DLIOM_HIP_TRY(hipStreamSynchronize(ctx->stream));
  {
    bool overflow = false;
    DLIOM_TRY(box_overflowed(ctx, err1, &overflow));
    if (overflow) {
      ctx->force_dense_score = true;
      const int s = run_score_volume(ctx, cloud, grid, c, 0, static_cast<int>(c.w.num_rotations), &d, &d_sums, &pad_processed);
      ctx->force_dense_score = false;
      DLIOM_TRY(s);
      DLIOM_HIP_TRY(hipMemcpyAsync(sums, d_sums, static_cast<size_t>(c.w.num_candidates) * 8, hipMemcpyDeviceToHost, ctx->stream));
      DLIOM_HIP_TRY(hipStreamSynchronize(ctx->stream));
    }
  }
  const uint64_t n_pad = static_cast<uint64_t>(pad_processed);
  for (int64_t i = 0; i < c.w.num_candidates; ++i) sums[i] -= n_pad;
  return DLIOM_OK;
}

int dliom_rtcsm3d_sequential_sums(dliom_ctx* ctx, const dliom_rtcsm_options* o, const double init7[7],
                                  const float* points_xyz, int64_t n, const dliom_grid* grid,
                                  const int64_t* candidate_indices, int64_t k, int method, float* sums) {
  if (ctx == nullptr || o == nullptr || init7 == nullptr || grid == nullptr || candidate_indices == nullptr ||
      sums == nullptr || n <= 0 || points_xyz == nullptr || k <= 0)
    return DLIOM_ERR_INVALID_ARGUMENT;
  DLIOM_HIP_TRY(hipSetDevice(ctx->device));
  DLIOM_TRY(ctx->points.reserve(staged_cloud_bytes(n)));
  dliom_cloud cloud;
  DLIOM_TRY(stage_cloud(ctx, points_xyz, n, &cloud));
  Candidates c;
  generate_candidates(*o, grid->resolution, cloud.max_norm, init7, &c);
  DeviceCandidates d;
  DLIOM_TRY(upload_candidates(ctx, c, &d));
  std::vector<unsigned> list(static_cast<size_t>(k));
  for (int64_t i = 0; i < k; ++i) {
    if (candidate_indices[i] < 0 || candidate_indices[i] >= c.w.num_candidates) return DLIOM_ERR_INVALID_ARGUMENT;
    list[i] = static_cast<unsigned>(candidate_indices[i]);
  }
  const size_t lbytes = align256(static_cast<size_t>(k) * 4);
  DLIOM_TRY(ctx->rescore.reserve(2 * lbytes));
  unsigned* d_list = ctx->rescore.as<unsigned>();
  float* d_ksums = reinterpret_cast<float*>(static_cast<char*>(ctx->rescore.p) + lbytes);
  DLIOM_HIP_TRY(hipMemcpyAsync(d_list, list.data(), static_cast<size_t>(k) * 4, hipMemcpyHostToDevice, ctx->stream));
  const int R = static_cast<int>(c.w.num_rotations);
  if (method < 0 || method > 2 || k > 65535) return DLIOM_ERR_INVALID_ARGUMENT;
  if (method != 0 && ((static_cast<size_t>(n) + 7) & ~static_cast<size_t>(7)) * 2 > 128 * 1024) return DLIOM_ERR_INVALID_ARGUMENT;
  DLIOM_TRY(launch_sequential_sums(ctx, method, grid->view(), cloud, d.rot, R, d.trans, d_list, nullptr,
                                   static_cast<unsigned>(k), &ctx->misc, d_ksums));
  DLIOM_HIP_TRY(hipMemcpyAsync(sums, d_ksums, static_cast<size_t>(k) * 4, hipMemcpyDeviceToHost, ctx->stream));
  DLIOM_HIP_TRY(hipStreamSynchronize(ctx->stream));
  return DLIOM_OK;
}

int dliom_probe_transform_cell_indices(dliom_ctx* ctx, const float pose[7], const float* points_xyz,
                                       int64_t n, float resolution, int32_t* cell_xyz) {
  if (ctx == nullptr || pose == nullptr || n < 0 || (n > 0 && (points_xyz == nullptr || cell_xyz == nullptr)))
    return DLIOM_ERR_INVALID_ARGUMENT;
  if (n == 0) return DLIOM_OK;
  DLIOM_HIP_TRY(hipSetDevice(ctx->device));
  DLIOM_TRY(ctx->points.reserve(staged_cloud_bytes(n)));
  dliom_cloud cloud;
  DLIOM_TRY(stage_cloud(ctx, points_xyz, n, &cloud));
  DLIOM_TRY(ctx->misc.reserve(static_cast<size_t>(n) * 12));
  int* d_out = ctx->misc.as<int>();
  const Quat4 q{pose[3], pose[4], pose[5], pose[6]};
  hipLaunchKernelGGL(probe_cells_kernel, dim3(static_cast<unsigned>((n + 255) / 256)), dim3(256), 0,
                     ctx->stream, q, pose[0], pose[1], pose[2], cloud.d_x, cloud.d_y, cloud.d_z,
                     static_cast<int>(n), resolution, d_out);
  DLIOM_HIP_TRY(hipGetLastError());
  DLIOM_HIP_TRY(hipMemcpyAsync(cell_xyz, d_out, static_cast<size_t>(n) * 12, hipMemcpyDeviceToHost,
                               ctx->stream));
  DLIOM_HIP_TRY(hipStreamSynchronize(ctx->stream));
  return DLIOM_OK;
}

}
```

Before: 983.9 scans/s.

## Streamline RTCSM host-side candidate and box-table preparation

Moves candidate generation into a header. Raw rotations are built from a single octant using sign symmetry and cached in SoA form, and the composed rotations are written straight into the pinned staging buffer, which removes the intermediate host vectors and copies. Box tables (tau, pass, bitmap) are also built in place in pinned memory. The per-group rotation spread now uses a series approximation for atan2 and only recomputes the exact value for candidates that can set the bounds. The changes target per-scan CPU overhead, but the slack-based pruning could in principle alter the bounds slightly and adds code complexity. Optional host timing instrumentation is included behind an experiments flag.

```diff
diff --git a/d-liom_amd/csrc/rtcsm3d.hip b/d-liom_amd/csrc/rtcsm3d.hip
--- a/d-liom_amd/csrc/rtcsm3d.hip
+++ b/d-liom_amd/csrc/rtcsm3d.hip
@@ -1,5 +1,6 @@
 #include <algorithm>
 #include <cmath>
+#include <cstdio>
 #include <cstdlib>
 #include <cstring>
 #include <type_traits>
@@ -11,6 +12,7 @@
 #include "device_common.h"
 #include "host_math.h"
 #include "probability_values.h"
+#include "rtcsm_candidates.h"
 #include "score_box.h"
 
 namespace dliom {
@@ -387,80 +389,6 @@
   out[3 * i + 2] = cell_of(rz + tz, resolution);
 }
 
-struct Candidates {
-  dliom_rtcsm_window w;
-  PoseF init;
-  std::vector<QF> rot;
-  std::vector<QF> rot_raw;
-  std::vector<float> r_angle;
-  std::vector<F3> trans;
-  std::vector<float> t_norm;
-};
-
-static void compute_window(const dliom_rtcsm_options& o, float resolution, float cloud_max_norm_value,
-                           dliom_rtcsm_window* w) {
-  w->linear_window_size = static_cast<int>(std::lround(o.linear_search_window / resolution));
-  float max_scan_range = 3.f * resolution;
-  max_scan_range = std::max(cloud_max_norm_value, max_scan_range);
-  const float kSafetyMargin = 1.f - 1e-3f;
-  const float res2 = resolution * (resolution * 1.f);
-  const float range2 = max_scan_range * (max_scan_range * 1.f);
-  w->angular_step_size = kSafetyMargin * std::acos(1.f - res2 / (2.f * range2));
-  w->angular_window_size =
-      static_cast<int>(std::lround(o.angular_search_window / w->angular_step_size));
-  w->max_scan_range = max_scan_range;
-  const int64_t tl = 2 * static_cast<int64_t>(w->linear_window_size) + 1;
-  const int64_t ta = 2 * static_cast<int64_t>(w->angular_window_size) + 1;
-  w->num_translations = tl * tl * tl;
-  w->num_rotations = ta * ta * ta;
-  w->num_candidates = w->num_translations * w->num_rotations;
-}
-
-static void generate_candidates(const dliom_rtcsm_options& o, float resolution, float max_norm,
-                                const double init7[7], Candidates* c) {
-  compute_window(o, resolution, max_norm, &c->w);
-  c->init.t = F3{static_cast<float>(init7[0]), static_cast<float>(init7[1]), static_cast<float>(init7[2])};
-  c->init.q = QF{static_cast<float>(init7[3]), static_cast<float>(init7[4]),
-                 static_cast<float>(init7[5]), static_cast<float>(init7[6])};
-  const int L = c->w.linear_window_size, A = c->w.angular_window_size;
-  const float step = c->w.angular_step_size;
-  struct RotCache {
-    int A = -1;
-    float step = 0.f;
-    std::vector<QF> rot_raw;
-    std::vector<float> r_angle;
-  };
-  static thread_local RotCache cache;
-  if (cache.A != A || cache.step != step) {
-    cache.A = A;
-    cache.step = step;
-    cache.rot_raw.clear();
-    cache.r_angle.clear();
-    cache.rot_raw.reserve(c->w.num_rotations);
-    cache.r_angle.reserve(c->w.num_rotations);
-    for (int rz = -A; rz <= A; ++rz)
-      for (int ry = -A; ry <= A; ++ry)
-        for (int rx = -A; rx <= A; ++rx) {
-          const QF q = angle_axis_to_quaternion(F3{rx * step, ry * step, rz * step});
-          cache.rot_raw.push_back(q);
-          cache.r_angle.push_back(rotation_angle(q));
-        }
-  }
-  c->rot_raw = cache.rot_raw;
-  c->r_angle = cache.r_angle;
-  c->rot.resize(cache.rot_raw.size());
-  for (size_t i = 0; i < cache.rot_raw.size(); ++i) c->rot[i] = qnormalized(qmul(c->init.q, cache.rot_raw[i]));
-  c->trans.clear();
-  c->t_norm.clear();
-  for (int z = -L; z <= L; ++z)
-    for (int y = -L; y <= L; ++y)
-      for (int x = -L; x <= L; ++x) {
-        const F3 t{x * resolution, y * resolution, z * resolution};
-        c->t_norm.push_back(norm3(t));
-        c->trans.push_back(add3(qrot(c->init.q, t), c->init.t));
-      }
-}
-
 struct DeviceCandidates {
   float4* rot;
   float* trans;
@@ -469,6 +397,34 @@
   float* r_angle;
   const float4* rot_src;
 };
+
+struct RtcsmState {
+  dliom_rtcsm_options o;
+  Candidates c;
+  DeviceCandidates d;
+  dliom_cloud cloud;
+  const dliom_grid* grid = nullptr;
+  int r_first = 0, r_last = 0;
+  unsigned long long* d_sums = nullptr;
+  float* d_hi = nullptr;
+  unsigned* d_list = nullptr;
+  unsigned* d_ctrs = nullptr;
+  float best_score = -1.f;
+  int64_t best_c = -1;
+  bool active = false;
+  double init7[7] = {0, 0, 0, 1, 0, 0, 0};
+  int shard = 0, num_shards = 1;
+  bool used_box = false;
+  std::vector<char> host_tables, host_box_tables;
+};
+
+static RtcsmState* state_of(dliom_ctx* ctx) {
+  if (ctx->rtcsm_state == nullptr) {
+    ctx->rtcsm_state = new RtcsmState;
+    ctx->rtcsm_state_free = [](void* p) { delete static_cast<RtcsmState*>(p); };
+  }
+  return static_cast<RtcsmState*>(ctx->rtcsm_state);
+}
 
 static bool prep_add(PrepArgs* prep, void* dst, const void* src, size_t bytes, unsigned value) {
   if (prep == nullptr || prep->n >= kMaxPrepJobs || (bytes & 3u) != 0 || (reinterpret_cast<uintptr_t>(dst) & 15u) != 0 ||
@@ -494,61 +450,59 @@
 }
 
 static int upload_candidates(dliom_ctx* ctx, const Candidates& c, DeviceCandidates* d, PrepArgs* prep = nullptr) {
-  const size_t R = c.rot.size(), T = c.trans.size();
-  const size_t Tpad = T;
-  const size_t bytes_rot = align256(R * 16);
-  const size_t bytes_trans = align256(Tpad * 12);
-  const size_t bytes_tn = align256(T * 4);
-  const size_t bytes_ra = align256(R * 4);
-  const size_t bytes_t4 = align256(T * 16);
-  const size_t total = bytes_rot + bytes_trans + bytes_tn + bytes_ra + bytes_t4;
-  DLIOM_TRY(ctx->cand.reserve(total));
-  std::vector<char> host(total, 0);
-  float* hr = reinterpret_cast<float*>(host.data());
-  for (size_t i = 0; i < R; ++i) {
-    hr[4 * i] = c.rot[i].w;
-    hr[4 * i + 1] = c.rot[i].x;
-    hr[4 * i + 2] = c.rot[i].y;
-    hr[4 * i + 3] = c.rot[i].z;
-  }
-  float* ht = reinterpret_cast<float*>(host.data() + bytes_rot);
-  for (size_t i = 0; i < Tpad; ++i) {
-    const F3& t = c.trans[std::min(i, T - 1)];
-    ht[3 * i] = t.x;
-    ht[3 * i + 1] = t.y;
-    ht[3 * i + 2] = t.z;
-  }
-  std::memcpy(host.data() + bytes_rot + bytes_trans, c.t_norm.data(), T * 4);
-  std::memcpy(host.data() + bytes_rot + bytes_trans + bytes_tn, c.r_angle.data(), R * 4);
-  float* h4 = reinterpret_cast<float*>(host.data() + bytes_rot + bytes_trans + bytes_tn + bytes_ra);
-  for (size_t i = 0; i < T; ++i) {
-    h4[4 * i] = c.trans[i].x;
-    h4[4 * i + 1] = c.trans[i].y;
-    h4[4 * i + 2] = c.trans[i].z;
-    h4[4 * i + 3] = 0.f;
-  }
+  const CandidateTableLayout l = candidate_table_layout(c.num_rotations(), c.trans.size());
+  DLIOM_TRY(ctx->cand.reserve(l.total));
   char* base = static_cast<char*>(ctx->cand.p);
   d->rot_src = reinterpret_cast<const float4*>(base);
-  if (total <= kPinRtcsmCandidates.bytes) {
-    void* staged = pinned_at(ctx, kPinRtcsmCandidates);
-    std::memcpy(staged, host.data(), total);
-    if (prep_add(prep, base, staged, total, 0u))
-      d->rot_src = static_cast<const float4*>(staged);
+  if (l.total <= kPinRtcsmCandidates.bytes) {
+    char* staged = pinned_at<char>(ctx, kPinRtcsmCandidates);
+    fill_candidate_tables(c, l, staged);
+    if (prep_add(prep, base, staged, l.total, 0u))
+      d->rot_src = reinterpret_cast<const float4*>(staged);
     else
-      DLIOM_HIP_TRY(hipMemcpyAsync(base, staged, total, hipMemcpyHostToDevice, ctx->stream));
+      DLIOM_HIP_TRY(hipMemcpyAsync(base, staged, l.total, hipMemcpyHostToDevice, ctx->stream));
   } else {
-    DLIOM_HIP_TRY(hipMemcpyAsync(base, host.data(), total, hipMemcpyHostToDevice, ctx->stream));
+    std::vector<char>& host = state_of(ctx)->host_tables;
+    host.resize(l.total);
+    fill_candidate_tables(c, l, host.data());
+    DLIOM_HIP_TRY(hipMemcpyAsync(base, host.data(), l.total, hipMemcpyHostToDevice, ctx->stream));
     DLIOM_HIP_TRY(hipStreamSynchronize(ctx->stream));
   }
-  d->rot = reinterpret_cast<float4*>(base);
-  d->trans = reinterpret_cast<float*>(base + bytes_rot);
-  d->t_norm = reinterpret_cast<float*>(base + bytes_rot + bytes_trans);
-  d->r_angle = reinterpret_cast<float*>(base + bytes_rot + bytes_trans + bytes_tn);
-  d->trans4 = reinterpret_cast<float4*>(base + bytes_rot + bytes_trans + bytes_tn + bytes_ra);
+  d->rot = reinterpret_cast<float4*>(base + l.rot);
+  d->trans = reinterpret_cast<float*>(base + l.trans);
+  d->t_norm = reinterpret_cast<float*>(base + l.t_norm);
+  d->r_angle = reinterpret_cast<float*>(base + l.r_angle);
+  d->trans4 = reinterpret_cast<float4*>(base + l.trans4);
   return DLIOM_OK;
 }
 
 static int env_int(const char* name, int fallback) { return tuning_int(name, fallback); }
+
+#ifdef DLIOM_EXPERIMENTS
+struct HostPrepClock {
+  static constexpr int kLaps = 6;
+  std::chrono::steady_clock::time_point t0;
+  std::vector<float> us[kLaps];
+  void start() { t0 = std::chrono::steady_clock::now(); }
+  void lap(int k) { us[k].push_back(std::chrono::duration<float, std::micro>(std::chrono::steady_clock::now() - t0).count()); }
+  void stop() { lap(kLaps - 1); }
+  ~HostPrepClock() {
+    std::vector<float>& total = us[kLaps - 1];
+    if (total.empty() || env_int("DLIOM_HOST_PREP_TIMING", 0) == 0) return;
+    double sum = 0.0;
+    for (float v : total) sum += v;
+    for (std::vector<float>& v : us) std::sort(v.begin(), v.end());
+    std::fprintf(stderr, "rtcsm host prep: matches %zu mean_us %.2f median_us %.2f min_us %.2f lap_medians_us", total.size(),
+                 sum / total.size(), total[total.size() / 2], total.front());
+    for (const std::vector<float>& v : us) std::fprintf(stderr, " %.2f", v.empty() ? 0.f : v[v.size() / 2]);
+    std::fprintf(stderr, "\n");
+  }
+};
+static HostPrepClock g_host_prep;
+#define DLIOM_PREP_LAP(k) g_host_prep.lap(k)
+#else
+#define DLIOM_PREP_LAP(k) ((void)0)
+#endif
 
 static int launch_score_box(dliom_ctx* ctx, const dliom_cloud& cloud, const GridView& g, const Candidates& c,
                             const DeviceCandidates& d, int r_first, int r_last, unsigned long long* d_sums,
@@ -573,8 +527,32 @@
   const double rmax = static_cast<double>(cloud.max_norm) / res + 1.0;
   const double qmax = rmax + tmax / res + 1.0;
   if (!std::isfinite(qmax) || qmax > 16500.0) return (ctx->last_box_refusal = DLIOM_BOX_REFUSED_RANGE, DLIOM_ERR_CAPACITY);
-  std::vector<Pass> pass(static_cast<size_t>(passes));
-  std::vector<float> tau(static_cast<size_t>(passes) * TC * 4, 0.f);
+  const int rot_groups_all = (r_last - r_first + 63) / 64;
+  static const int forced_nw = env_int("DLIOM_BOX_NW", 0);
+  const int nw = forced_nw >= 1 && forced_nw <= kWaves
+                     ? std::min(forced_nw, rot_groups_all)
+                     : std::min(rot_groups_all, kWaves);
+  const int rot_blocks = (rot_groups_all + nw - 1) / nw;
+  const size_t tau_count = static_cast<size_t>(passes) * TC * 4, bitmap_count = static_cast<size_t>(passes) * kBitmapWords;
+  const size_t tau_bytes = align256(tau_count * 4);
+  const size_t pass_only_bytes = align256(static_cast<size_t>(passes) * sizeof(Pass));
+  const size_t group_bytes = align256(static_cast<size_t>(rot_blocks) * sizeof(Group));
+  const size_t bitmap_bytes = align256(bitmap_count * 4);
+  const size_t pass_bytes = pass_only_bytes + group_bytes + bitmap_bytes;
+  const bool tables_staged = tau_bytes + pass_bytes <= kPinBoxTables.bytes;
+  char* h = nullptr;
+  if (tables_staged) {
+    h = pinned_at<char>(ctx, kPinBoxTables);
+  } else {
+    std::vector<char>& host = state_of(ctx)->host_box_tables;
+    host.resize(tau_bytes + pass_bytes);
+    h = host.data();
+  }
+  float* const tau = reinterpret_cast<float*>(h);
+  Pass* const pass = reinterpret_cast<Pass*>(h + tau_bytes);
+  unsigned* const bitmap = reinterpret_cast<unsigned*>(h + tau_bytes + pass_only_bytes + group_bytes);
+  std::memset(tau, 0, tau_count * 4);
+  std::memset(pass, 0, static_cast<size_t>(passes) * sizeof(Pass));
   double taumax = 0.0;
   for (int tp = 0; tp < passes; ++tp) {
     const int j0 = tp * TC, tc = std::min(TC, T - j0);
@@ -623,12 +601,12 @@
       ps.reach[a] = static_cast<float>(reach + 0.02 + qmax * std::ldexp(1.0, -22));
     }
   }
-  std::vector<unsigned> bitmap(static_cast<size_t>(passes) * kBitmapWords, 0u);
+  std::memset(bitmap, 0, bitmap_count * 4);
   const unsigned thr_units = static_cast<unsigned>(s_units + B);
   for (int tp = 0; tp < passes; ++tp) {
     const Pass& ps = pass[static_cast<size_t>(tp)];
     for (int a = 0; a < 3; ++a) {
-      unsigned* words = bitmap.data() + static_cast<size_t>(tp) * kBitmapWords + static_cast<size_t>(a) * (kBuckets / 32);
+      unsigned* words = bitmap + static_cast<size_t>(tp) * kBitmapWords + static_cast<size_t>(a) * (kBuckets / 32);
       for (int jj = 0; jj < ps.tc; ++jj) {
         const double tv = static_cast<double>(tau[(static_cast<size_t>(tp) * TC + jj) * 4 + a]);
         const double af = tv - std::floor(tv);
@@ -648,12 +626,6 @@
     const double dim = spread + 2.0 * taumax + 8.0;
     if (dim > kMaxDim || dim * dim * (dim * 0.25) > cells) return (ctx->last_box_refusal = DLIOM_BOX_REFUSED_WINDOW, DLIOM_ERR_CAPACITY);
   }
-  const int rot_groups_all = (r_last - r_first + 63) / 64;
-  static const int forced_nw = env_int("DLIOM_BOX_NW", 0);
-  const int nw = forced_nw >= 1 && forced_nw <= kWaves
-                     ? std::min(forced_nw, rot_groups_all)
-                     : std::min(rot_groups_all, kWaves);
-  const int rot_blocks = (rot_groups_all + nw - 1) / nw;
   if (TC * sizeof(float4) + kBitmapWords * 4 + 16 + static_cast<size_t>(nw) * kListWords * 4 + static_cast<size_t>(cells) * 2 >
       160 * 1024)
     return (ctx->last_box_refusal = DLIOM_BOX_REFUSED_LDS, DLIOM_ERR_CAPACITY);
@@ -681,35 +653,13 @@
       gr.c_lane = 0;
       continue;
     }
-    auto qd = [&](int r, double q[4]) {
-      const QF& f = c.rot_raw[static_cast<size_t>(r)];
-      const double nn = std::sqrt(double(f.w) * f.w + double(f.x) * f.x + double(f.y) * f.y + double(f.z) * f.z);
-      q[0] = f.w / nn; q[1] = f.x / nn; q[2] = f.y / nn; q[3] = f.z / nn;
-    };
-    double qc[4];
-    qd(r0 + gr.c_lane, qc);
-    double lo3[3] = {1e300, 1e300, 1e300}, hi3[3] = {-1e300, -1e300, -1e300}, th = 0.0;
-    for (int l = 0; l < cnt; ++l) {
-      double q[4];
-      qd(r0 + l, q);
-      const double a0 = qc[0], a1 = -qc[1], a2 = -qc[2], a3 = -qc[3];
-      double dq[4] = {a0 * q[0] - a1 * q[1] - a2 * q[2] - a3 * q[3], a0 * q[1] + a1 * q[0] + a2 * q[3] - a3 * q[2],
-                      a0 * q[2] - a1 * q[3] + a2 * q[0] + a3 * q[1], a0 * q[3] + a1 * q[2] - a2 * q[1] + a3 * q[0]};
-      if (dq[0] < 0) for (double& v : dq) v = -v;
-      const double vn = std::sqrt(dq[1] * dq[1] + dq[2] * dq[2] + dq[3] * dq[3]);
-      const double ang = 2.0 * std::atan2(vn, dq[0]);
-      const double k = vn > 1e-300 ? ang / vn : 2.0;
-      const double dv[3] = {k * dq[1], k * dq[2], k * dq[3]};
-      th = std::max(th, ang);
-      for (int a = 0; a < 3; ++a) {
-        lo3[a] = std::min(lo3[a], dv[a]);
-        hi3[a] = std::max(hi3[a], dv[a]);
-      }
-    }
+    RotationSpread sp;
+    rotation_spread(c, r0, cnt, &sp);
+    const double th = sp.max_angle;
     if (th > 0.3) return (ctx->last_box_refusal = DLIOM_BOX_REFUSED_WINDOW, DLIOM_ERR_CAPACITY);
     for (int a = 0; a < 3; ++a) {
-      gr.dc[a] = static_cast<float>(0.5 * (lo3[a] + hi3[a]));
-      gr.hd[a] = static_cast<float>(0.5 * (hi3[a] - lo3[a]) * 1.0001 + 1e-7);
+      gr.dc[a] = static_cast<float>(0.5 * (sp.lo[a] + sp.hi[a]));
+      gr.hd[a] = static_cast<float>(0.5 * (sp.hi[a] - sp.lo[a]) * 1.0001 + 1e-7);
     }
     gr.theta2 = static_cast<float>(0.51 * th * th * 1.01 + 1e-9);
   }
@@ -718,36 +668,24 @@
   gcache.r_first = r_first;
   gcache.r_last = r_last;
   gcache.nw = nw;
+  DLIOM_PREP_LAP(3);
   struct SpanGuard {
     dliom_ctx* c;
     int span;
     ~SpanGuard() { c->end_span(span); }
   } span_guard{ctx, ctx->begin_span(DLIOM_KERNEL_RTCSM_SCORE)};
-  const size_t tau_bytes = align256(tau.size() * 4);
-  const size_t pass_only_bytes = align256(pass.size() * sizeof(Pass));
-  const size_t group_bytes = align256(groups.size() * sizeof(Group));
-  const size_t bitmap_bytes = align256(bitmap.size() * 4);
-  const size_t pass_bytes = pass_only_bytes + group_bytes + bitmap_bytes;
+  DLIOM_PREP_LAP(4);
   DLIOM_TRY(ctx->box_tables.reserve(tau_bytes + pass_bytes));
   char* base = static_cast<char*>(ctx->box_tables.p);
   const Group* group_src = reinterpret_cast<const Group*>(base + tau_bytes + pass_only_bytes);
-  if (tau_bytes + pass_bytes <= kPinBoxTables.bytes) {
-    char* h = pinned_at<char>(ctx, kPinBoxTables);
-    std::memcpy(h, tau.data(), tau.size() * 4);
-    std::memcpy(h + tau_bytes, pass.data(), pass.size() * sizeof(Pass));
-    std::memcpy(h + tau_bytes + pass_only_bytes, groups.data(), groups.size() * sizeof(Group));
-    std::memcpy(h + tau_bytes + pass_only_bytes + group_bytes, bitmap.data(), bitmap.size() * 4);
+  std::memcpy(h + tau_bytes + pass_only_bytes, groups.data(), groups.size() * sizeof(Group));
+  if (tables_staged) {
     if (prep_add(prep, base, h, tau_bytes + pass_bytes, 0u))
       group_src = reinterpret_cast<const Group*>(h + tau_bytes + pass_only_bytes);
     else
       DLIOM_HIP_TRY(hipMemcpyAsync(base, h, tau_bytes + pass_bytes, hipMemcpyHostToDevice, ctx->stream));
   } else {
-    DLIOM_HIP_TRY(hipMemcpyAsync(base, tau.data(), tau.size() * 4, hipMemcpyHostToDevice, ctx->stream));
-    DLIOM_HIP_TRY(hipMemcpyAsync(base + tau_bytes, pass.data(), pass.size() * sizeof(Pass), hipMemcpyHostToDevice, ctx->stream));
-    DLIOM_HIP_TRY(hipMemcpyAsync(base + tau_bytes + pass_only_bytes, groups.data(), groups.size() * sizeof(Group),
-                                 hipMemcpyHostToDevice, ctx->stream));
-    DLIOM_HIP_TRY(hipMemcpyAsync(base + tau_bytes + pass_only_bytes + group_bytes, bitmap.data(), bitmap.size() * 4,
-                                 hipMemcpyHostToDevice, ctx->stream));
+    DLIOM_HIP_TRY(hipMemcpyAsync(base, h, tau_bytes + pass_bytes, hipMemcpyHostToDevice, ctx->stream));
     DLIOM_HIP_TRY(hipStreamSynchronize(ctx->stream));
   }
   Params p;
@@ -814,6 +752,9 @@
   p.ext_stride = static_cast<int>(cloud.n_padded);
   DLIOM_TRY(ctx->box_extents.reserve(static_cast<size_t>(rot_blocks) * 6 * static_cast<size_t>(cloud.n_padded) * 4));
   p.ext = ctx->box_extents.as<float>();
+#ifdef DLIOM_EXPERIMENTS
+  g_host_prep.stop();
+#endif
   {
     PrepArgs none;
     none.n = 0;
@@ -961,6 +902,7 @@
   PrepArgs prep;
   prep.n = 0;
   DLIOM_TRY(upload_candidates(ctx, c, d, &prep));
+  DLIOM_PREP_LAP(1);
   const int64_t C = c.w.num_candidates;
   DLIOM_TRY(ctx->sums.reserve(static_cast<size_t>(C) * 8));
   *d_sums = ctx->sums.as<unsigned long long>();
@@ -995,6 +937,7 @@
   if (windowed && mapping == 2) mapping = 1;
   const GridView g = grid->view();
   DLIOM_TRY(ensure_morton(ctx, &cloud));
+  DLIOM_PREP_LAP(2);
   if (g.log2_leaves > 10 && mapping >= 1) {
     if (mapping == 3) ctx->last_box_refusal = DLIOM_BOX_REFUSED_NO_MIRROR;
     mapping = 0;
@@ -1059,25 +1002,6 @@
   return m;
 }
 
-struct RtcsmState {
-  dliom_rtcsm_options o;
-  Candidates c;
-  DeviceCandidates d;
-  dliom_cloud cloud;
-  const dliom_grid* grid = nullptr;
-  int r_first = 0, r_last = 0;
-  unsigned long long* d_sums = nullptr;
-  float* d_hi = nullptr;
-  unsigned* d_list = nullptr;
-  unsigned* d_ctrs = nullptr;
-  float best_score = -1.f;
-  int64_t best_c = -1;
-  bool active = false;
-  double init7[7] = {0, 0, 0, 1, 0, 0, 0};
-  int shard = 0, num_shards = 1;
-  bool used_box = false;
-};
-
 static int box_overflowed(dliom_ctx* ctx, unsigned err1, bool* overflow) {
   *overflow = err1 != 0u;
   if (*overflow)
@@ -1085,17 +1009,12 @@
   return DLIOM_OK;
 }
 
-static RtcsmState* state_of(dliom_ctx* ctx) {
-  if (ctx->rtcsm_state == nullptr) {
-    ctx->rtcsm_state = new RtcsmState;
-    ctx->rtcsm_state_free = [](void* p) { delete static_cast<RtcsmState*>(p); };
-  }
-  return static_cast<RtcsmState*>(ctx->rtcsm_state);
-}
-
 static int match_begin(dliom_ctx* ctx, const dliom_rtcsm_options* o, const double init7[7],
                        const dliom_cloud& cloud, const dliom_grid* grid, int shard, int num_shards,
                        unsigned* local_best_lo_bits) {
+#ifdef DLIOM_EXPERIMENTS
+  g_host_prep.start();
+#endif
   if (cloud.n <= 0) return DLIOM_ERR_EMPTY_CLOUD;
   if (cloud.n > (1 << 27) || num_shards < 1 || shard < 0 || shard >= num_shards)
     return DLIOM_ERR_INVALID_ARGUMENT;
@@ -1110,6 +1029,7 @@
   st->used_box = false;
   Candidates& c = st->c;
   generate_candidates(*o, grid->resolution, cloud.max_norm, init7, &c);
+  DLIOM_PREP_LAP(0);
   const int64_t C = c.w.num_candidates;
   const int R = static_cast<int>(c.w.num_rotations), T = static_cast<int>(c.w.num_translations);
   if (C <= 0 || C > (int64_t{1} << 31)) return DLIOM_ERR_INVALID_ARGUMENT;
@@ -1298,10 +1218,11 @@
   out7[0] = c.trans[j].x;
   out7[1] = c.trans[j].y;
   out7[2] = c.trans[j].z;
-  out7[3] = c.rot[r].w;
-  out7[4] = c.rot[r].x;
-  out7[5] = c.rot[r].y;
-  out7[6] = c.rot[r].z;
+  const QF q = c.rot(static_cast<size_t>(r));
+  out7[3] = q.w;
+  out7[4] = q.x;
+  out7[5] = q.y;
+  out7[6] = q.z;
   *out_score = score;
   ctx->last_rtcsm.best_index = best_c;
   return DLIOM_OK;
diff --git a/d-liom_amd/csrc/rtcsm_candidates.h b/d-liom_amd/csrc/rtcsm_candidates.h
--- /dev/null
+++ b/d-liom_amd/csrc/rtcsm_candidates.h
@@ -0,0 +1,247 @@
+#ifndef DLIOM_CSRC_RTCSM_CANDIDATES_H_
+#define DLIOM_CSRC_RTCSM_CANDIDATES_H_
+
+#include <algorithm>
+#include <cmath>
+#include <cstddef>
+#include <cstdint>
+#include <cstdlib>
+#include <cstring>
+#include <vector>
+
+#include "../../include/dliom.h"
+#include "host_math.h"
+
+namespace dliom {
+
+struct Candidates {
+  dliom_rtcsm_window w;
+  PoseF init;
+  int table_A = -1;
+  float table_step = 0.f;
+  std::vector<float> raw_w, raw_x, raw_y, raw_z;
+  std::vector<float> r_angle;
+  std::vector<QF> octant_q;
+  std::vector<float> octant_angle;
+  std::vector<double> octant_unit;
+  std::vector<double> unit_raw;
+  std::vector<F3> trans;
+  std::vector<float> t_norm;
+  size_t num_rotations() const { return r_angle.size(); }
+  QF rot_raw(size_t r) const { return QF{raw_w[r], raw_x[r], raw_y[r], raw_z[r]}; }
+  QF rot(size_t r) const { return qnormalized(qmul(init.q, rot_raw(r))); }
+};
+
+inline void compute_window(const dliom_rtcsm_options& o, float resolution, float cloud_max_norm_value,
+                           dliom_rtcsm_window* w) {
+  w->linear_window_size = static_cast<int>(std::lround(o.linear_search_window / resolution));
+  float max_scan_range = 3.f * resolution;
+  max_scan_range = std::max(cloud_max_norm_value, max_scan_range);
+  const float kSafetyMargin = 1.f - 1e-3f;
+  const float res2 = resolution * (resolution * 1.f);
+  const float range2 = max_scan_range * (max_scan_range * 1.f);
+  w->angular_step_size = kSafetyMargin * std::acos(1.f - res2 / (2.f * range2));
+  w->angular_window_size =
+      static_cast<int>(std::lround(o.angular_search_window / w->angular_step_size));
+  w->max_scan_range = max_scan_range;
+  const int64_t tl = 2 * static_cast<int64_t>(w->linear_window_size) + 1;
+  const int64_t ta = 2 * static_cast<int64_t>(w->angular_window_size) + 1;
+  w->num_translations = tl * tl * tl;
+  w->num_rotations = ta * ta * ta;
+  w->num_candidates = w->num_translations * w->num_rotations;
+}
+
+#if defined(__GNUC__) && !defined(__clang__)
+__attribute__((optimize("fp-contract=off")))
+#endif
+inline void compose_rotations(const QF& a, const float* __restrict__ bw, const float* __restrict__ bx,
+                              const float* __restrict__ by, const float* __restrict__ bz, size_t n, float* __restrict__ out4) {
+#if defined(__clang__)
+#pragma clang fp contract(off)
+#endif
+  const float aw = a.w, ax = a.x, ay = a.y, az = a.z;
+  for (size_t i = 0; i < n; ++i) {
+    const float x = (ax * bw[i] - az * by[i]) + (ay * bz[i] + aw * bx[i]);
+    const float y = (ay * bw[i] - ax * bz[i]) + (az * bx[i] + aw * by[i]);
+    const float z = (az * bw[i] - ay * bx[i]) + (ax * by[i] + aw * bz[i]);
+    const float w = (aw * bw[i] - ax * bx[i]) - (az * bz[i] + ay * by[i]);
+    const float z2 = (x * x + z * z) + (y * y + w * w);
+    const float len = std::sqrt(z2);
+    const bool scale = z2 > 0.f;
+    out4[4 * i] = scale ? w / len : w;
+    out4[4 * i + 1] = scale ? x / len : x;
+    out4[4 * i + 2] = scale ? y / len : y;
+    out4[4 * i + 3] = scale ? z / len : z;
+  }
+}
+
+inline void generate_candidates(const dliom_rtcsm_options& o, float resolution, float max_norm, const double init7[7],
+                                Candidates* c) {
+  compute_window(o, resolution, max_norm, &c->w);
+  c->init.t = F3{static_cast<float>(init7[0]), static_cast<float>(init7[1]), static_cast<float>(init7[2])};
+  c->init.q = QF{static_cast<float>(init7[3]), static_cast<float>(init7[4]),
+                 static_cast<float>(init7[5]), static_cast<float>(init7[6])};
+  const int L = c->w.linear_window_size, A = c->w.angular_window_size;
+  const float step = c->w.angular_step_size;
+  if (c->table_A != A || c->table_step != step || c->r_angle.size() != static_cast<size_t>(c->w.num_rotations)) {
+    c->table_A = -1;
+    const size_t A1 = static_cast<size_t>(A) + 1;
+    c->octant_q.resize(A1 * A1 * A1);
+    c->octant_angle.resize(A1 * A1 * A1);
+    c->octant_unit.resize(4 * A1 * A1 * A1);
+    c->unit_raw.resize(4 * static_cast<size_t>(c->w.num_rotations));
+    for (int rz = 0; rz <= A; ++rz)
+      for (int ry = 0; ry <= A; ++ry)
+        for (int rx = 0; rx <= A; ++rx) {
+          const size_t k = (static_cast<size_t>(rz) * A1 + ry) * A1 + rx;
+          c->octant_q[k] = angle_axis_to_quaternion(F3{rx * step, ry * step, rz * step});
+          c->octant_angle[k] = rotation_angle(c->octant_q[k]);
+          const QF& f = c->octant_q[k];
+          const double nn = std::sqrt(double(f.w) * f.w + double(f.x) * f.x + double(f.y) * f.y + double(f.z) * f.z);
+          const double unit[4] = {f.w / nn, f.x / nn, f.y / nn, f.z / nn};
+          std::memcpy(&c->octant_unit[4 * k], unit, sizeof unit);
+        }
+    for (std::vector<float>* v : {&c->raw_w, &c->raw_x, &c->raw_y, &c->raw_z, &c->r_angle})
+      v->resize(static_cast<size_t>(c->w.num_rotations));
+    size_t r = 0;
+    for (int rz = -A; rz <= A; ++rz)
+      for (int ry = -A; ry <= A; ++ry)
+        for (int rx = -A; rx <= A; ++rx, ++r) {
+          const size_t k = (static_cast<size_t>(std::abs(rz)) * A1 + std::abs(ry)) * A1 + std::abs(rx);
+          const QF& q = c->octant_q[k];
+          c->raw_w[r] = q.w;
+          c->raw_x[r] = rx < 0 ? -q.x : q.x;
+          c->raw_y[r] = ry < 0 ? -q.y : q.y;
+          c->raw_z[r] = rz < 0 ? -q.z : q.z;
+          c->r_angle[r] = c->octant_angle[k];
+          const double* u = &c->octant_unit[4 * k];
+          double* out = &c->unit_raw[4 * r];
+          out[0] = u[0];
+          out[1] = rx < 0 ? -u[1] : u[1];
+          out[2] = ry < 0 ? -u[2] : u[2];
+          out[3] = rz < 0 ? -u[3] : u[3];
+        }
+    c->table_A = A;
+    c->table_step = step;
+  }
+  c->trans.clear();
+  c->t_norm.clear();
+  for (int z = -L; z <= L; ++z)
+    for (int y = -L; y <= L; ++y)
+      for (int x = -L; x <= L; ++x) {
+        const F3 t{x * resolution, y * resolution, z * resolution};
+        c->t_norm.push_back(norm3(t));
+        c->trans.push_back(add3(qrot(c->init.q, t), c->init.t));
+      }
+}
+
+struct RotationSpread {
+  double lo[3], hi[3], max_angle;
+};
+inline void rotation_spread(const Candidates& c, int r0, int cnt, RotationSpread* out) {
+  constexpr double kSlack = 1e-9, kSeriesMax = 0.2;
+  static thread_local std::vector<double> scratch;
+  scratch.resize(9 * static_cast<size_t>(cnt));
+  double *d0 = scratch.data(), *d1 = d0 + cnt, *d2 = d1 + cnt, *d3 = d2 + cnt, *vn = d3 + cnt, *ang = vn + cnt;
+  double *v1 = ang + cnt, *v2 = v1 + cnt, *v3 = v2 + cnt;
+  const double* u = &c.unit_raw[4 * static_cast<size_t>(r0)];
+  const double* qc = u + 4 * static_cast<size_t>(cnt / 2);
+  const double a0 = qc[0], a1 = -qc[1], a2 = -qc[2], a3 = -qc[3];
+  for (int l = 0; l < cnt; ++l) {
+    const double* q = u + 4 * static_cast<size_t>(l);
+    const double e0 = a0 * q[0] - a1 * q[1] - a2 * q[2] - a3 * q[3], e1 = a0 * q[1] + a1 * q[0] + a2 * q[3] - a3 * q[2];
+    const double e2 = a0 * q[2] - a1 * q[3] + a2 * q[0] + a3 * q[1], e3 = a0 * q[3] + a1 * q[2] - a2 * q[1] + a3 * q[0];
+    const bool flip = e0 < 0;
+    d0[l] = flip ? -e0 : e0;
+    d1[l] = flip ? -e1 : e1;
+    d2[l] = flip ? -e2 : e2;
+    d3[l] = flip ? -e3 : e3;
+    vn[l] = std::sqrt(d1[l] * d1[l] + d2[l] * d2[l] + d3[l] * d3[l]);
+  }
+  const auto exact_angle = [&](int l) { return 2.0 * std::atan2(vn[l], d0[l]); };
+  for (int l = 0; l < cnt; ++l) {
+    const double t = vn[l] / d0[l], s = t * t;
+    ang[l] = 2.0 * (t * (1.0 + s * (-1.0 / 3 + s * (1.0 / 5 + s * (-1.0 / 7 + s * (1.0 / 9 + s * (-1.0 / 11 + s * (1.0 / 13))))))));
+  }
+  double low_of_hi[3] = {-1e300, -1e300, -1e300}, high_of_lo[3] = {1e300, 1e300, 1e300}, low_of_angle = 0.0;
+  for (int l = 0; l < cnt; ++l) {
+    if (!(vn[l] > 1e-300 && vn[l] <= kSeriesMax * d0[l])) ang[l] = exact_angle(l);
+    const double k = vn[l] > 1e-300 ? ang[l] / vn[l] : 2.0;
+    v1[l] = k * d1[l];
+    v2[l] = k * d2[l];
+    v3[l] = k * d3[l];
+    const double v[3] = {v1[l], v2[l], v3[l]};
+    for (int a = 0; a < 3; ++a) {
+      const double slack = std::fabs(v[a]) * kSlack;
+      low_of_hi[a] = std::max(low_of_hi[a], v[a] - slack);
+      high_of_lo[a] = std::min(high_of_lo[a], v[a] + slack);
+    }
+    low_of_angle = std::max(low_of_angle, ang[l] * (1.0 - kSlack));
+  }
+  for (int a = 0; a < 3; ++a) {
+    out->lo[a] = 1e300;
+    out->hi[a] = -1e300;
+  }
+  out->max_angle = 0.0;
+  for (int l = 0; l < cnt; ++l) {
+    const double v[3] = {v1[l], v2[l], v3[l]};
+    bool decides = ang[l] * (1.0 + kSlack) >= low_of_angle;
+    for (int a = 0; a < 3; ++a) {
+      const double slack = std::fabs(v[a]) * kSlack;
+      decides = decides || v[a] + slack >= low_of_hi[a] || v[a] - slack <= high_of_lo[a];
+    }
+    if (!decides) continue;
+    const double angle = exact_angle(l);
+    const double k = vn[l] > 1e-300 ? angle / vn[l] : 2.0;
+    const double dv[3] = {k * d1[l], k * d2[l], k * d3[l]};
+    out->max_angle = std::max(out->max_angle, angle);
+    for (int a = 0; a < 3; ++a) {
+      out->lo[a] = std::min(out->lo[a], dv[a]);
+      out->hi[a] = std::max(out->hi[a], dv[a]);
+    }
+  }
+}
+
+struct CandidateTableLayout {
+  size_t rot = 0, trans = 0, t_norm = 0, r_angle = 0, trans4 = 0, total = 0;
+};
+inline CandidateTableLayout candidate_table_layout(size_t R, size_t T) {
+  const auto up = [](size_t bytes) { return (bytes + 255) & ~static_cast<size_t>(255); };
+  CandidateTableLayout l;
+  l.trans = l.rot + up(R * 16);
+  l.t_norm = l.trans + up(T * 12);
+  l.r_angle = l.t_norm + up(T * 4);
+  l.trans4 = l.r_angle + up(R * 4);
+  l.total = l.trans4 + up(T * 16);
+  return l;
+}
+
+inline void fill_candidate_tables(const Candidates& c, const CandidateTableLayout& l, char* dst) {
+  const size_t R = c.num_rotations(), T = c.trans.size();
+  const auto pad = [dst](size_t from, size_t to) { std::memset(dst + from, 0, to - from); };
+  compose_rotations(c.init.q, c.raw_w.data(), c.raw_x.data(), c.raw_y.data(), c.raw_z.data(), R,
+                    reinterpret_cast<float*>(dst + l.rot));
+  pad(l.rot + R * 16, l.trans);
+  float* ht = reinterpret_cast<float*>(dst + l.trans);
+  float* h4 = reinterpret_cast<float*>(dst + l.trans4);
+  for (size_t i = 0; i < T; ++i) {
+    const F3& t = c.trans[i];
+    ht[3 * i] = t.x;
+    ht[3 * i + 1] = t.y;
+    ht[3 * i + 2] = t.z;
+    h4[4 * i] = t.x;
+    h4[4 * i + 1] = t.y;
+    h4[4 * i + 2] = t.z;
+    h4[4 * i + 3] = 0.f;
+  }
+  pad(l.trans + T * 12, l.t_norm);
+  std::memcpy(dst + l.t_norm, c.t_norm.data(), T * 4);
+  pad(l.t_norm + T * 4, l.r_angle);
+  std::memcpy(dst + l.r_angle, c.r_angle.data(), R * 4);
+  pad(l.r_angle + R * 4, l.trans4);
+  pad(l.trans4 + T * 16, l.total);
+}
+
+}
+
+#endif
```

Measured after the change: 1015 scans/s (median of 6 runs). 1.03x the previous value.
